# xxxupeng/stereo_toolbox

Measured on AMD Instinct MI355X. Metric: stereo pairs/sec @ 540x960 D=192 (GwcNet_GC fwd+bwd), higher is better.
Workload: dtype f32; 1 GPU; GwcNet_GC(maxdisp=192) train step: fwd+bwd+allreduce+Adam, 576x960 pairs (reference pad_to_2x shape), batch 1/GPU, fp32, synthetic randn inputs, deterministic filler weights; global_batch=1, parallelism=dp1, grad_sync=none (single rank: flat fp32 buffer packed, no collective), launch=eager, optimizer=torch.optim.Adam(fused=True)

## Files before the change

include/stx_hip.h:

```cpp
#ifndef STX_HIP_H
#define STX_HIP_H
#ifdef __cplusplus
extern "C" {
#endif

const char* stx_last_error(void);
const char* stx_build_info(void);
int stx_get_tuning(const char* name);
int stx_set_tuning(const char* name, int value);

int stx_cost_volume_fwd(const float* Lg, const float* Rg, int Cg, int G, const float* Lc, const float* Rc, int Cc,
                        const float* scale, float* vol, int B, int H, int W, int D, int mask_left, void* stream);
int stx_group_normalize_fwd(const float* x, float* y, int B, int C, int G, int HW, float out_scale, void* stream);
int stx_group_normalize_bwd(const float* x, const float* gy, float* gx, int B, int C, int G, int HW, float out_scale, void* stream);
int stx_cost_volume_bwd(const float* gvol, const float* Lg, const float* Rg, int Cg, int G, int Cc, float* gLg,
                        float* gRg, float* gLc, float* gRc, int B, int H, int W, int D, int mask_left, void* stream);

int stx_head_fwd(const float* cost, float* disp, float* stats, int B, int Dc, int Hc, int Wc, int D, int H, int W,
                 void* stream);
long long stx_head_bwd_workspace_floats(int B, int Dc, int H, int W);
int stx_head_bwd(const float* gdisp, const float* cost, const float* disp, const float* stats, float* gcost,
                 float* workspace, int B, int Dc, int Hc, int Wc, int D, int H, int W, void* stream);
int stx_head_fwd2(const float* cost, float* disp, float* stats, int B, int Dc, int Hc, int Wc, int D, int H, int W,
                  int align_corners, void* stream);
int stx_head_bwd2(const float* gdisp, const float* cost, const float* disp, const float* stats, float* gcost,
                  float* workspace, int B, int Dc, int Hc, int Wc, int D, int H, int W, int align_corners, void* stream);
int stx_softargmax_fwd(const float* x, float* out, int B, int D, int HW, void* stream);
int stx_argmax_fwd(const float* x, long long* out, int B, int D, int HW, void* stream);
int stx_unimodal_fwd(const float* x, float* out, int B, int D, int HW, void* stream);
int stx_dominant_modal_fwd(const float* x, float* out, int B, int D, int HW, void* stream);
int stx_modal_fwd(const float* x, float* out, float* aux, int B, int D, int HW, int kind, void* stream);
int stx_modal_bwd(const float* g, const float* out, const float* aux, float* gx, int B, int D, int HW, void* stream);
int stx_split_mode(const float* x, float* mode, unsigned char* mask, int B, int D, int HW, void* stream);
int stx_softmax_d_fwd(const float* x, float* y, int B, int D, int HW, void* stream);

long long stx_conv3d_packed_floats(int K, int N, int T);
int stx_conv3d_pack_weight(const float* w, float* wp, int A, int B, int T, int mode, void* stream);
int stx_conv3d_fwd_blocks(int Do, int Ho, int Wo);
long long stx_conv3d_fwd_stat_rows(int B, int Di, int Hi, int Wi, int Cin, int Cout, int ks, int stride);
int stx_conv3d_fwd(const float* x, const float* wp, float* out, const float* scale, const float* bias,
                   const float* residual, float* stats, int B, int Di, int Hi, int Wi, int Cin, int Cout, int ks,
                   int stride, int relu, void* stream);
int stx_deconv3d_fwd_blocks(int Di, int Hi, int Wi);
int stx_deconv3d_fwd(const float* x, const float* wp, float* out, const float* scale, const float* bias,
                     const float* residual, float* stats, int B, int Di, int Hi, int Wi, int Cin, int Cout, int Do,
                     int Ho, int Wo, int relu, void* stream);
long long stx_conv3d_wgrad_workspace_floats(int B, int Dc, int Hc, int Wc, int CF, int CC, int ks, int stride);
int stx_conv3d_wgrad(const float* fine, const float* coarse, float* dw, float* workspace, int B, int Df, int Hf, int Wf,
                     int CF, int Dc, int Hc, int Wc, int CC, int ks, int stride, void* stream);

int stx_conv3d_wgrad_bn_supported(int B, int D, int H, int W, int CF, int CC);
int stx_conv3d_wgrad_bn(const float* x, const float* gy, const float* z, const float* scale, const float* shift, const float* mean,
                        const float* invstd, const float* gamma, const float* sums, float inv_n, int act, float* dz, float* dw,
                        float* workspace, int B, int D, int H, int W, int CF, int CC, void* stream);

int stx_conv2d_supported(int Cin, int Cout);
long long stx_conv2d_stat_rows(int groups);
int stx_conv2d_fwd(const float* x, const float* w, float* out, float* stats, int B, int H, int W, int Cin, int Cout, int dgrad,
                   int groups, void* stream);

int stx_conv3d_c1_fwd(const float* x, const float* w, const float* residual, float* out, int B, int D, int H, int W,
                      int Cin, void* stream);
long long stx_conv3d_c1_wgrad_workspace_floats(int Cin);
int stx_conv3d_c1_wgrad(const float* x, const float* gy, float* dw, float* workspace, int B, int D, int H, int W,
                        int Cin, void* stream);
int stx_conv3d_c1_dgrad(const float* gy, const float* w, float* gx, int B, int D, int H, int W, int Cin, void* stream);

int stx_mish_fwd(const float* x, float* y, long long n, void* stream);
int stx_mish_bwd(const float* gy, const float* x, float* gx, long long n, void* stream);
int stx_depth_to_space(const float* y, float* out, int B, int D, int H, int W, int C, int inverse, void* stream);
int stx_gate_fwd(const float* cv, const float* att, float* out, int B, int D, long long HW, int C, void* stream);
int stx_gate_bwd(const float* g, const float* cv, const float* att, float* gcv, float* gatt, int B, int D, long long HW,
                 int C, void* stream);

int stx_concat_channels(const float* in0, const float* in1, const float* in2, const float* in3, int C0, int C1, int C2, int C3,
                        float* out, long long nvox, void* stream);
int stx_split_channels(const float* in, float* out0, float* out1, float* out2, float* out3, int C0, int C1, int C2, int C3,
                       long long nvox, void* stream);
int stx_transpose(const float* in, float* out, int N, int rows, int cols, void* stream);

int stx_dwconv_hw_fwd(const float* x, const float* w, const int* dil, float* out, int B, int D, int H, int W, int C,
                      int flip, void* stream);
long long stx_dwconv_hw_wgrad_workspace_floats(int C);
int stx_dwconv_hw_wgrad(const float* x, const float* gy, const int* dil, float* dw, float* workspace, int B, int D,
                        int H, int W, int C, void* stream);
int stx_cost_volume_scale_bwd(const float* gvol, const float* Lc, const float* Rc, float* gscale, int B, int Cc, int H,
                              int W, int D, int mask_left, void* stream);
int stx_scale_channels(const float* x, const float* s, float* out, long long nvox, int C, void* stream);
int stx_ac_volume_bwd(const float* gvol, const float* Lc, const float* Rc, const float* prob, float* gL, float* gR,
                      float* gprob, int B, int Cc, int H, int W, int D, int mask_left, void* stream);

int stx_bn_reduce_blocks(void);
int stx_bn_stats_rows(long long nvox, int C);
int stx_bn_stats(const float* z, float* partials, long long nvox, int C, int groups, void* stream);
int stx_bn_finalize(const float* partials, int nrows, int C, double count, const float* gamma, const float* beta,
                    float* running_mean, float* running_var, float momentum, float eps, float* scale, float* shift,
                    float* mean, float* invstd, void* stream);
int stx_bn_finalize_groups(const float* partials, int nrows, int C, double count, const float* gamma, const float* beta,
                           float* running_mean, float* running_var, float momentum, float eps, float* out, int groups,
                           void* stream);
int stx_bn_apply(const float* z1, const float* scale1, const float* shift1, const float* z2, const float* scale2,
                 const float* shift2, float* out, long long nvox, int C, int relu, int groups, void* stream);
int stx_bn_bwd_reduce(const float* gy, const float* y, const float* z1, const float* mean1, const float* invstd1,
                      const float* z2, const float* mean2, const float* invstd2, float* partials, float* sums,
                      long long nvox, int C, int relu, void* stream);
int stx_bn_bwd_apply(const float* gy, const float* y, const float* z1, const float* mean1, const float* invstd1,
                     const float* gamma1, const float* z2, const float* mean2, const float* invstd2,
                     const float* gamma2, const float* sums, float* dz1, float* dz2, float* gout, long long nvox, int C,
                     int relu, void* stream);
int stx_bn_bwd_reduce2(const float* gy, const float* y, const float* z1, const float* mean1, const float* invstd1,
                       const float* z2, const float* mean2, const float* invstd2, const float* scale1,
                       const float* shift1, const float* scale2, const float* shift2, float* partials, float* sums,
                       long long nvox, int C, int relu, int groups, void* stream);
int stx_bn_bwd_apply2(const float* gy, const float* y, const float* z1, const float* mean1, const float* invstd1,
                      const float* gamma1, const float* z2, const float* mean2, const float* invstd2,
                      const float* gamma2, const float* scale1, const float* shift1, const float* scale2,
                      const float* shift2, const float* sums, float* dz1, float* dz2, float* gout, long long nvox,
                      int C, int relu, int groups, void* stream);

int stx_pad_normalize_u8(const unsigned char* img, float* out, int B, int H, int W, int Hp, int Wp, int top,
                         const float* mean3, const float* std3, void* stream);

int stx_sampled_volume_fwd(const float* Lg, const float* Rg, int Cg, int G, const float* Lc, const float* Rc, int Cc,
                           const float* samples, float* vol, int B, int H, int W, int S, int CTp, void* stream);
int stx_sampled_volume_bwd(const float* gvol, const float* Lg, const float* Rg, int Cg, int G, int Cc,
                           const float* samples, float* gLg, float* gRg, float* gLc, float* gRc, int B, int H, int W,
                           int S, int CTp, void* stream);

int stx_warp_fwd(const float* x, const float* disp, float* out, int B, int C, int H, int W, void* stream);
int stx_warp_bwd(const float* gout, const float* x, const float* disp, float* gx, float* gdisp, int B, int C, int H, int W,
                 void* stream);
int stx_corr_volume_fwd(const float* ref, const float* tgt, float* vol, int B, int C, int H, int W, int maxdisp, int groups,
                        void* stream);
int stx_corr_volume_bwd(const float* gvol, const float* ref, const float* tgt, float* gref, float* gtgt, int B, int C, int H,
                        int W, int maxdisp, int groups, void* stream);
int stx_disparity_variance_fwd(const float* x, const float* disp, const float* samples, float* out, int B, int D, int HW,
                               void* stream);
int stx_disparity_variance_bwd(const float* g, const float* x, const float* disp, const float* samples, float* gx, float* gdisp,
                               float* gsamples, int B, int D, int HW, void* stream);

long long stx_geo_pyramid_floats(long long rows, int len, int C, int levels);
int stx_geo_corr_fwd(const float* fmap1, const float* fmap2, float* cpyr, int B, int C, int H, int W1, int W2, int levels,
                     void* stream);
int stx_geo_corr_bwd(const float* gcpyr, const float* fmap1, const float* fmap2, float* gfmap1, float* gfmap2, int B, int C, int H,
                     int W1, int W2, int levels, void* stream);
int stx_geo_pyramid_fwd(const float* vol, float* gpyr, int B, int D, int H, int W, int C, int levels, void* stream);
int stx_geo_pyramid_bwd(const float* ggpyr, float* gvol, int B, int D, int H, int W, int C, int levels, void* stream);
int stx_geo_lookup_fwd(const float* gpyr, const float* cpyr, const float* disp, const float* coords, float* out, int B, int H,
                       int W, int D, int C, int W2, int levels, int radius, void* stream);
int stx_geo_lookup_bwd(const float* gout, const float* disp, const float* coords, float* ggpyr, float* gcpyr, int B, int H, int W,
                       int D, int C, int W2, int levels, int radius, void* stream);
int stx_context_upsample_fwd(const float* disp_low, const float* up_weights, float* out, int B, int h, int w, void* stream);
int stx_context_upsample_bwd(const float* g, const float* disp_low, const float* up_weights, float* gdisp, float* gweights, int B,
                             int h, int w, void* stream);

long long stx_corr1d_pyramid_floats(long long rows, int W2, int levels);
int stx_corr1d_pyramid_fwd(const float* fmap1, const float* fmap2, float* cpyr, int B, int C, int H, int W1, int W2, int levels,
                           float scale, void* stream);
int stx_corr1d_pyramid_bwd(const float* gcpyr, const float* fmap1, const float* fmap2, float* gfmap1, float* gfmap2, int B, int C,
                           int H, int W1, int W2, int levels, float scale, void* stream);
int stx_corr1d_lookup_fwd(const float* cpyr, const float* base, const float* disp, const float* jobs, int njobs, float* out, int B,
                          int H, int W1, int W2, int levels, void* stream);
int stx_corr1d_lookup_bwd(const float* gout, const float* base, const float* disp, const float* jobs, int njobs, float* gcpyr,
                          int B, int H, int W1, int W2, int levels, void* stream);

int stx_allpairs_estimates_fwd(const float* vol, int which, float* disp_l, float* conf_l, float* disp_r, float* conf_r, float* stats,
                               int B, int H, int W1, int W2, void* stream);
int stx_allpairs_estimates_bwd(const float* g_disp_l, const float* g_conf_l, const float* g_disp_r, const float* g_conf_r,
                               const float* vol, const float* stats, float* gvol, int B, int H, int W1, int W2, void* stream);
int stx_corr1d_volume_pyramid_fwd(const float* vol, const float* tdisp, const float* tconf, float atten, float* cpyr, int B, int H,
                                  int W1, int W2, int levels, void* stream);
int stx_corr1d_volume_pyramid_bwd(const float* gcpyr, const float* tdisp, const float* tconf, float atten, float* gvol, int B, int H,
                                  int W1, int W2, int levels, void* stream);
int stx_truncate_mask_fwd(const float* disp, const float* conf, int has_th, float conf_th, float atten, float* mask, int B, int H,
                          int W, void* stream);

int stx_photo_warp_fwd(const float* right, const float* disp, float* warped, float* valid, int B, int C, int H, int W, void* stream);
int stx_photo_warp_bwd(const float* gwarped, const float* right, const float* disp, float* gdisp, int B, int C, int H, int W,
                       void* stream);
int stx_ssim_fwd(const float* x, const float* y, float* out, int B, int C, int H, int W, int window, void* stream);
long long stx_ssim_bwd_workspace_floats(int B, int C, int H, int W);
int stx_ssim_bwd(const float* g_out, const float* x, const float* y, float* gx, float* gy, float* workspace, int B, int C, int H, int W,
                 int window, void* stream);
int stx_photometric_fwd(const float* left, const float* right, const float* disp, double ssim_weight, int enable_mask, float* loss,
                        int B, int C, int H, int W, void* stream);
long long stx_photometric_bwd_workspace_floats(int B, int C, int H, int W);
int stx_photometric_bwd(const float* gloss, const float* left, const float* right, const float* disp, double ssim_weight,
                        int enable_mask, float* gdisp, float* workspace, int B, int C, int H, int W, void* stream);
int stx_auto_mask_fwd(const float* left, const float* right, const float* disp, int denorm, unsigned char* mask, int B, int C, int H,
                      int W, void* stream);
long long stx_smoothness_workspace_floats(int B, int H, int W);
int stx_smoothness_fwd(const float* disp, const float* img, float* out, float* stats, float* workspace, int B, int C, int H, int W,
                       void* stream);
int stx_smoothness_bwd(const float* gout, const float* disp, const float* img, const float* stats, float* gdisp, int B, int C, int H,
                       int W, void* stream);

int stx_sttr_head_fwd(const float* attn, const float* phi, int mode, int iters, float log_one, float log_bin, float log_2w,
                      const unsigned char* occ_mask, const float* target, float* disp, float* occ, float* norm, int* arg,
                      float* gt_response, float* bin_left, float* bin_right, double* us, double* vs, int N, int H, int W, void* stream);
int stx_sttr_head_bwd(const float* g_disp, const float* g_occ, const float* g_gt, const float* g_bin_left, const float* g_bin_right,
                      const float* attn, const float* phi, int mode, int iters, float log_one, float log_bin, float log_2w,
                      const float* target, const float* disp, const float* norm, const int* arg, const double* us, const double* vs,
                      float* g_attn, double* phi_partials, float* g_phi, int N, int H, int W, void* stream);
int stx_sttr_transport_fwd(const float* attn, const float* phi, int mode, int iters, float log_one, float log_bin, float log_2w,
                           float* P, double* us, double* vs, int N, int H, int W, void* stream);
int stx_sttr_transport_bwd(const float* G, const float* attn, const float* phi, int mode, int iters, float log_one, float log_bin,
                           float log_2w, const double* us, const double* vs, float* g_attn, double* phi_partials, float* g_phi, int N,
                           int H, int W, void* stream);

#ifdef __cplusplus
}
#endif
#endif
```

stereo_toolbox_amd/_capi.py:

```python
import ctypes
import os
import threading

import torch

_P = ctypes.c_void_p
_I = ctypes.c_int
_F = ctypes.c_float
_L = ctypes.c_longlong

SIGNATURES = {
    "stx_get_tuning": [ctypes.c_char_p],
    "stx_set_tuning": [ctypes.c_char_p, _I],
    "stx_cost_volume_fwd": [_P, _P, _I, _I, _P, _P, _I, _P, _P, _I, _I, _I, _I, _I, _P],
    "stx_cost_volume_bwd": [_P, _P, _P, _I, _I, _I, _P, _P, _P, _P, _I, _I, _I, _I, _I, _P],
    "stx_group_normalize_fwd": [_P, _P, _I, _I, _I, _I, _F, _P],
    "stx_group_normalize_bwd": [_P, _P, _P, _I, _I, _I, _I, _F, _P],
    "stx_head_fwd": [_P, _P, _P, _I, _I, _I, _I, _I, _I, _I, _P],
    "stx_head_bwd_workspace_floats": [_I, _I, _I, _I],
    "stx_head_bwd": [_P, _P, _P, _P, _P, _P, _I, _I, _I, _I, _I, _I, _I, _P],
    "stx_head_fwd2": [_P, _P, _P, _I, _I, _I, _I, _I, _I, _I, _I, _P],
    "stx_head_bwd2": [_P, _P, _P, _P, _P, _P, _I, _I, _I, _I, _I, _I, _I, _I, _P],
    "stx_softargmax_fwd": [_P, _P, _I, _I, _I, _P],
    "stx_argmax_fwd": [_P, _P, _I, _I, _I, _P],
    "stx_softmax_d_fwd": [_P, _P, _I, _I, _I, _P],
    "stx_unimodal_fwd": [_P, _P, _I, _I, _I, _P],
    "stx_dominant_modal_fwd": [_P, _P, _I, _I, _I, _P],
    "stx_modal_fwd": [_P, _P, _P, _I, _I, _I, _I, _P],
    "stx_modal_bwd": [_P, _P, _P, _P, _I, _I, _I, _P],
    "stx_split_mode": [_P, _P, _P, _I, _I, _I, _P],
    "stx_conv3d_packed_floats": [_I, _I, _I],
    "stx_conv3d_pack_weight": [_P, _P, _I, _I, _I, _I, _P],
    "stx_conv3d_fwd_blocks": [_I, _I, _I],
    "stx_conv3d_fwd_stat_rows": [_I, _I, _I, _I, _I, _I, _I, _I],
    "stx_deconv3d_fwd_blocks": [_I, _I, _I],
    "stx_conv3d_fwd": [_P, _P, _P, _P, _P, _P, _P, _I, _I, _I, _I, _I, _I, _I, _I, _I, _P],
    "stx_deconv3d_fwd": [_P, _P, _P, _P, _P, _P, _P, _I, _I, _I, _I, _I, _I, _I, _I, _I, _I, _P],
    "stx_conv3d_wgrad_workspace_floats": [_I, _I, _I, _I, _I, _I, _I, _I],
    "stx_conv3d_wgrad": [_P, _P, _P, _P, _I, _I, _I, _I, _I, _I, _I, _I, _I, _I, _I, _P],
    "stx_conv3d_wgrad_bn_supported": [_I, _I, _I, _I, _I, _I],
    "stx_conv3d_wgrad_bn": [_P] * 9 + [_F, _I, _P, _P, _P, _I, _I, _I, _I, _I, _I, _P],
    "stx_conv2d_supported": [_I, _I],
    "stx_conv2d_stat_rows": [_I],
    "stx_conv2d_fwd": [_P, _P, _P, _P, _I, _I, _I, _I, _I, _I, _I, _P],
    "stx_conv3d_c1_fwd": [_P, _P, _P, _P, _I, _I, _I, _I, _I, _P],
    "stx_conv3d_c1_wgrad_workspace_floats": [_I],
    "stx_conv3d_c1_wgrad": [_P, _P, _P, _P, _I, _I, _I, _I, _I, _P],
    "stx_conv3d_c1_dgrad": [_P, _P, _P, _I, _I, _I, _I, _I, _P],
    "stx_mish_fwd": [_P, _P, _L, _P],
    "stx_mish_bwd": [_P, _P, _P, _L, _P],
    "stx_depth_to_space": [_P, _P, _I, _I, _I, _I, _I, _I, _P],
    "stx_gate_fwd": [_P, _P, _P, _I, _I, _L, _I, _P],
    "stx_gate_bwd": [_P, _P, _P, _P, _P, _I, _I, _L, _I, _P],
    "stx_concat_channels": [_P, _P, _P, _P, _I, _I, _I, _I, _P, _L, _P],
    "stx_split_channels": [_P, _P, _P, _P, _P, _I, _I, _I, _I, _L, _P],
    "stx_transpose": [_P, _P, _I, _I, _I, _P],
    "stx_dwconv_hw_fwd": [_P, _P, _P, _P, _I, _I, _I, _I, _I, _I, _P],
    "stx_dwconv_hw_wgrad_workspace_floats": [_I],
    "stx_dwconv_hw_wgrad": [_P, _P, _P, _P, _P, _I, _I, _I, _I, _I, _P],
    "stx_cost_volume_scale_bwd": [_P, _P, _P, _P, _I, _I, _I, _I, _I, _I, _P],
    "stx_scale_channels": [_P, _P, _P, _L, _I, _P],
    "stx_ac_volume_bwd": [_P, _P, _P, _P, _P, _P, _P, _I, _I, _I, _I, _I, _I, _P],
    "stx_pad_normalize_u8": [_P, _P, _I, _I, _I, _I, _I, _I, _P, _P, _P],
    "stx_warp_fwd": [_P, _P, _P, _I, _I, _I, _I, _P],
    "stx_warp_bwd": [_P, _P, _P, _P, _P, _I, _I, _I, _I, _P],
    "stx_corr_volume_fwd": [_P, _P, _P, _I, _I, _I, _I, _I, _I, _P],
    "stx_corr_volume_bwd": [_P, _P, _P, _P, _P, _I, _I, _I, _I, _I, _I, _P],
    "stx_disparity_variance_fwd": [_P, _P, _P, _P, _I, _I, _I, _P],
    "stx_disparity_variance_bwd": [_P, _P, _P, _P, _P, _P, _P, _I, _I, _I, _P],
    "stx_sampled_volume_fwd": [_P, _P, _I, _I, _P, _P, _I, _P, _P, _I, _I, _I, _I, _I, _P],
    "stx_sampled_volume_bwd": [_P, _P, _P, _I, _I, _I, _P, _P, _P, _P, _P, _I, _I, _I, _I, _I, _P],
    "stx_geo_pyramid_floats": [_L, _I, _I, _I],
    "stx_geo_corr_fwd": [_P, _P, _P, _I, _I, _I, _I, _I, _I, _P],
    "stx_geo_corr_bwd": [_P, _P, _P, _P, _P, _I, _I, _I, _I, _I, _I, _P],
    "stx_geo_pyramid_fwd": [_P, _P, _I, _I, _I, _I, _I, _I, _P],
    "stx_geo_pyramid_bwd": [_P, _P, _I, _I, _I, _I, _I, _I, _P],
    "stx_geo_lookup_fwd": [_P, _P, _P, _P, _P, _I, _I, _I, _I, _I, _I, _I, _I, _P],
    "stx_geo_lookup_bwd": [_P, _P, _P, _P, _P, _I, _I, _I, _I, _I, _I, _I, _I, _P],
    "stx_context_upsample_fwd": [_P, _P, _P, _I, _I, _I, _P],
    "stx_context_upsample_bwd": [_P, _P, _P, _P, _P, _I, _I, _I, _P],
    "stx_corr1d_pyramid_floats": [_L, _I, _I],
    "stx_corr1d_pyramid_fwd": [_P, _P, _P, _I, _I, _I, _I, _I, _I, _F, _P],
    "stx_corr1d_pyramid_bwd": [_P, _P, _P, _P, _P, _I, _I, _I, _I, _I, _I, _F, _P],
    "stx_corr1d_lookup_fwd": [_P, _P, _P, _P, _I, _P, _I, _I, _I, _I, _I, _P],
    "stx_corr1d_lookup_bwd": [_P, _P, _P, _P, _I, _P, _I, _I, _I, _I, _I, _P],
    "stx_allpairs_estimates_fwd": [_P, _I, _P, _P, _P, _P, _P, _I, _I, _I, _I, _P],
    "stx_allpairs_estimates_bwd": [_P, _P, _P, _P, _P, _P, _P, _I, _I, _I, _I, _P],
    "stx_corr1d_volume_pyramid_fwd": [_P, _P, _P, _F, _P, _I, _I, _I, _I, _I, _P],
    "stx_corr1d_volume_pyramid_bwd": [_P, _P, _P, _F, _P, _I, _I, _I, _I, _I, _P],
    "stx_truncate_mask_fwd": [_P, _P, _I, _F, _F, _P, _I, _I, _I, _P],
    "stx_photo_warp_fwd": [_P, _P, _P, _P, _I, _I, _I, _I, _P],
    "stx_photo_warp_bwd": [_P, _P, _P, _P, _I, _I, _I, _I, _P],
    "stx_ssim_fwd": [_P, _P, _P, _I, _I, _I, _I, _I, _P],
    "stx_ssim_bwd_workspace_floats": [_I, _I, _I, _I],
    "stx_ssim_bwd": [_P, _P, _P, _P, _P, _P, _I, _I, _I, _I, _I, _P],
    "stx_photometric_fwd": [_P, _P, _P, ctypes.c_double, _I, _P, _I, _I, _I, _I, _P],
    "stx_photometric_bwd_workspace_floats": [_I, _I, _I, _I],
    "stx_photometric_bwd": [_P, _P, _P, _P, ctypes.c_double, _I, _P, _P, _I, _I, _I, _I, _P],
    "stx_auto_mask_fwd": [_P, _P, _P, _I, _P, _I, _I, _I, _I, _P],
    "stx_smoothness_workspace_floats": [_I, _I, _I],
    "stx_smoothness_fwd": [_P, _P, _P, _P, _P, _I, _I, _I, _I, _P],
    "stx_smoothness_bwd": [_P, _P, _P, _P, _P, _I, _I, _I, _I, _P],
    "stx_sttr_head_fwd": [_P, _P, _I, _I, _F, _F, _F] + [_P] * 11 + [_I, _I, _I, _P],
    "stx_sttr_head_bwd": [_P] * 7 + [_I, _I, _F, _F, _F] + [_P] * 9 + [_I, _I, _I, _P],
    "stx_sttr_transport_fwd": [_P, _P, _I, _I, _F, _F, _F, _P, _P, _P, _I, _I, _I, _P],
    "stx_sttr_transport_bwd": [_P, _P, _P, _I, _I, _F, _F, _F, _P, _P, _P, _P, _P, _I, _I, _I, _P],
    "stx_bn_reduce_blocks": [],
    "stx_bn_stats_rows": [_L, _I],
    "stx_bn_stats": [_P, _P, _L, _I, _I, _P],
    "stx_bn_finalize": [_P, _I, _I, ctypes.c_double, _P, _P, _P, _P, _F, _F, _P, _P, _P, _P, _P],
    "stx_bn_finalize_groups": [_P, _I, _I, ctypes.c_double, _P, _P, _P, _P, _F, _F, _P, _I, _P],
    "stx_bn_apply": [_P, _P, _P, _P, _P, _P, _P, _L, _I, _I, _I, _P],
    "stx_bn_bwd_reduce": [_P, _P, _P, _P, _P, _P, _P, _P, _P, _P, _L, _I, _I, _P],
    "stx_bn_bwd_apply": [_P, _P, _P, _P, _P, _P, _P, _P, _P, _P, _P, _P, _P, _P, _L, _I, _I, _P],
    "stx_bn_bwd_reduce2": [_P] * 14 + [_L, _I, _I, _I, _P],
    "stx_bn_bwd_apply2": [_P] * 18 + [_L, _I, _I, _I, _P],
}
_RET_CHARP = ("stx_last_error", "stx_build_info")


class StxError(RuntimeError):
    pass


class StxLib:

    def __init__(self, path):
        if not os.path.exists(path):
            raise StxError(
                f"HIP library not found: {path}. Build it with `python -m stereo_toolbox_amd.build` "
                "(hipcc, gfx950). There is no CPU fallback for the cost-volume hot path.")
        self.path = path
        self._dll = ctypes.CDLL(path)
        for name in _RET_CHARP:
            fn = getattr(self._dll, name)
            fn.restype = ctypes.c_char_p
            fn.argtypes = []
        self._fns = {}
        for name, argtypes in SIGNATURES.items():
            fn = getattr(self._dll, name, None)
            if fn is None:
                continue
            fn.restype = ctypes.c_longlong if name.endswith(("_floats", "_stat_rows")) else _I
            fn.argtypes = argtypes
            self._fns[name] = fn

    def has(self, name):
        return name in self._fns

    def build_info(self):
        return self._dll.stx_build_info().decode()

    def get_tuning(self, name):
        return self._fns["stx_get_tuning"](name.encode())

    def set_tuning(self, name, value):
        old = self.get_tuning(name)
        if old < 0 or self._fns["stx_set_tuning"](name.encode(), int(value)) != 0:
            raise StxError(f"unknown tuning switch {name}")
        return old

    def raw(self, name):
        return self._fns[name]

    def call(self, name, *args):
        fn = self._fns.get(name)
        if fn is None:
            raise StxError(f"{self.path} does not export {name}")
        rc = fn(*args)
        if rc != 0:
            raise StxError(f"{name} failed ({rc}): {self._dll.stx_last_error().decode()}")


_LIB = None
_LOCK = threading.Lock()
LIB_PATH = os.environ.get("STX_HIP_LIB") or os.path.join(os.path.dirname(os.path.abspath(__file__)), "lib", "libstx_hip.so")


def get_lib():
    global _LIB
    if _LIB is None:
        with _LOCK:
            if _LIB is None:
                _LIB = StxLib(LIB_PATH)
    return _LIB
```

stereo_toolbox_amd/aggregation.py:

```python
import os
import threading

import torch
import torch.nn as nn

from . import ops


def _is_transposed(conv):
    return isinstance(conv, nn.ConvTranspose3d)


def _conv_cfg(conv):
    ks = conv.kernel_size[0]
    stride = conv.stride[0]
    if _is_transposed(conv):
        k3 = ks == 3 and stride == 2 and conv.padding[0] == 1 and conv.output_padding[0] == 1
        k4 = ks == 4 and stride == 2 and conv.padding[0] == 1 and conv.output_padding[0] == 0
        if not (k3 or k4) or len(set(conv.kernel_size)) != 1 or len(set(conv.stride)) != 1:
            raise ops.StxError("only ConvTranspose3d(k=3, s=2, p=1, op=1) and ConvTranspose3d(k=4, s=2, p=1) are on the hot path")
    else:
        if not ((ks == 3 and conv.padding[0] == 1 and stride in (1, 2)) or (ks == 1 and conv.padding[0] == 0 and stride == 1)):
            raise ops.StxError(f"unsupported Conv3d k={ks} s={stride} p={conv.padding}")
    if conv.bias is not None or conv.groups != 1:
        raise ops.StxError("hot-path convolutions are bias-free and dense")
    return ks, stride


def _fold(bn):
    key = (bn.weight._version, bn.bias._version, bn.running_mean._version, bn.running_var._version,
           bn.weight.data_ptr(), bn.bias.data_ptr(), bn.running_mean.data_ptr(), bn.running_var.data_ptr())
    hit = bn.__dict__.get("_stx_fold") if ops._CACHE_ENABLED else None
    if hit is not None and hit[0] == key:
        return hit[1], hit[2]
    with torch.no_grad():
        scale = (bn.weight * torch.rsqrt(bn.running_var + bn.eps)).contiguous()
        bias = (bn.bias - bn.running_mean * scale).contiguous()
    if ops._CACHE_ENABLED:
        bn.__dict__["_stx_fold"] = (key, scale, bias)
    return scale, bias


def _needs_grad(*tensors_and_modules):
    if not torch.is_grad_enabled():
        return False
    for t in tensors_and_modules:
        if t is None:
            continue
        if isinstance(t, torch.Tensor):
            if t.requires_grad:
                return True
        else:
            if any(p.requires_grad for p in t.parameters()):
                return True
    return False


def _infer_conv(x, conv, scale, bias, residual, relu):
    ks, stride = _conv_cfg(conv)
    if _is_transposed(conv) and ks == 4:
        if residual is not None:
            raise ops.StxError("ConvTranspose3d(k4) with a fused residual is not wired (no model uses it)")
        return ops.deconv4_forward(x, conv.weight.detach(), scale, bias, int(relu), owner=conv.weight)
    if _is_transposed(conv):
        wp = ops.pack_weight(conv.weight.detach(), 2, owner=conv.weight)
        return ops.deconv3d_forward(x, wp, conv.weight.shape[1], scale=scale, bias=bias, residual=residual, relu=relu)[0]
    if ops._is_c1(conv.weight, ks, stride, False) and scale is None and bias is None and not relu:
        return ops.conv3d_c1_forward(x, conv.weight.detach().contiguous(), residual)
    if x.shape[-1] != conv.weight.shape[1]:
        if x.shape[-1] != (conv.weight.shape[1] + 7) // 8 * 8:
            raise ops.StxError(f"conv: input has {x.shape[-1]} channels, weight expects {conv.weight.shape[1]}")
        wpad = ops.pad_weight_channels(conv.weight.detach(), x.shape[-1])
        return ops.conv3d_forward(x, ops.pack_weight(wpad, 0), conv.weight.shape[0], ks, stride, scale, bias, residual, relu)[0]
    if x.shape[-1] % 8 != 0:
        xp, wpad = ops.pad_input_channels(x, conv.weight.detach())
        return ops.conv3d_forward(xp, ops.pack_weight(wpad, 0), conv.weight.shape[0], ks, stride, scale, bias, residual, relu)[0]
    wp = ops.pack_weight(conv.weight.detach(), 0, owner=conv.weight)
    return ops.conv3d_forward(x, wp, conv.weight.shape[0], ks, stride, scale, bias, residual, relu)[0]


class deferred_bn_counters:
    _tls = threading.local()

    @staticmethod
    def _state():
        st = deferred_bn_counters._tls
        if not hasattr(st, "active"):
            st.active, st.pending = 0, []
        return st

    def __enter__(self):
        self._state().active += 1
        ops.bn_defer_reset_if_stale()
        return self

    def __exit__(self, *exc):
        st = self._state()
        st.active -= 1
        if st.active == 0 and st.pending:
            pend, st.pending = st.pending, []
            by_dev = {}
            for t in pend:
                d = by_dev.setdefault(t.device, {})
                ent = d.setdefault(id(t), [t, 0])
                ent[1] += 1
            for d in by_dev.values():
                torch._foreach_add_([e[0] for e in d.values()], [e[1] for e in d.values()])
        return False


def _bn_state(bn, partials, count, steps=1):
    training = bn.training
    sync = None
    if training and isinstance(bn, nn.SyncBatchNorm):
        import torch.distributed as dist
        if dist.is_available() and dist.is_initialized() and dist.get_world_size(bn.process_group) > 1:
            sync = (bn.process_group, dist.get_world_size(bn.process_group))
    if training:
        bn.__dict__.pop("_stx_fold", None)
    if training and bn.track_running_stats and bn.num_batches_tracked is not None:
        st = deferred_bn_counters._state()
        if st.active and bn.momentum is not None:
            st.pending.extend([bn.num_batches_tracked] * steps)
        else:
            bn.num_batches_tracked.add_(steps)
    if bn.momentum is not None:
        momentum = bn.momentum
    elif training and bn.track_running_stats and bn.num_batches_tracked is not None:
        momentum = 1.0 / float(bn.num_batches_tracked.item())
    else:
        momentum = 0.0
    return {"training": training, "partials": partials, "count": count, "running_mean": bn.running_mean,
            "running_var": bn.running_var, "momentum": momentum, "eps": bn.eps, "sync": sync}


def _raw_conv(x, conv, want):
    ks, stride = _conv_cfg(conv)
    if _is_transposed(conv) and ks == 4:
        return ops.deconv4_raw(x, conv.weight, want)
    return ops.ConvRawFn.apply(x, conv.weight, ks, stride, _is_transposed(conv), want)


@ops.fp32_region
def shared_input_convs(x, blocks):
    cfgs, ws = [], []
    for seq in blocks:
        conv, bn = seq[0], seq[1]
        if _is_transposed(conv) or not bn.training or conv.weight.shape[1] != x.shape[-1] or conv.weight.shape[1] % 8 \
                or conv.weight.shape[0] % 8:
            return None
        ks, stride = _conv_cfg(conv)
        cfgs.append((ks, stride, True))
        ws.append(conv.weight)
    if not _needs_grad(x, *[m for seq in blocks for m in (seq[0], seq[1])]):
        return None
    outs = ops.SharedInputConvsFn.apply(x, tuple(cfgs), *ws)
    return [(outs[2 * k], outs[2 * k + 1]) for k in range(len(blocks))]


@ops.fp32_region
def conv_block(x, conv, bn=None, relu=False, second=None, residual=None, mish=False, leaky=False, raw=None, second_raw=None):
    if (mish and relu) or (leaky and (relu or mish)):
        raise ops.StxError("conv_block: relu, mish and leaky are mutually exclusive")
    if second is not None and residual is not None:
        raise ops.StxError("conv_block: `second` and `residual` are mutually exclusive")
    mods = [conv, bn] + ([second[1], second[2]] if second is not None else [])
    grad = (raw is not None or second_raw is not None
            or _needs_grad(x, residual, *(m for m in mods if m is not None), *([second[0]] if second else [])))
    train_bn = (bn is not None and bn.training) or (second is not None and second[2].training)
    if mish and (grad or train_bn) and (bn is None or residual is not None):
        return ops.mish(conv_block(x, conv, bn, relu=False, second=second, residual=residual))
    if mish:
        relu = 2
    if leaky:
        relu = 3

    if not grad and not train_bn:
        if second is not None:
            s2, b2 = _fold(second[2])
            residual = _infer_conv(second[0], second[1], s2, b2, None, False)
        if bn is not None:
            s1, b1 = _fold(bn)
        else:
            s1 = b1 = None
        return _infer_conv(x, conv, s1, b1, residual, relu)

    want = bn is not None and bn.training
    z1, part1 = raw if raw is not None else _raw_conv(x, conv, want)
    if bn is None:
        y = z1
        if residual is not None:
            y = y + residual
        if relu == 3:
            return torch.nn.functional.leaky_relu(y, 0.01)
        return torch.relu(y) if relu else y
    count1 = z1.numel() // z1.shape[-1]
    st1 = _bn_state(bn, part1 if want else None, count1)
    if second is not None:
        x2, conv2, bn2 = second
        want2 = bn2.training
        z2, part2 = second_raw if second_raw is not None else _raw_conv(x2, conv2, want2)
        st2 = _bn_state(bn2, part2 if want2 else None, z2.numel() // z2.shape[-1])
        return ops.BnActFn.apply(z1, bn.weight, bn.bias, z2, bn2.weight, bn2.bias, None, relu, st1, st2)
    defer = (residual is None and want and relu in (0, 1, False, True) and not _is_transposed(conv) and _conv_cfg(conv) == (3, 1)
             and conv.weight.shape[0] % 32 == 0 and conv.weight.shape[1] % 32 == 0 and not st1.get("sync")
             and os.environ.get("STX_BN_BWD_IN_WGRAD", "1") != "0")
    if defer:
        ops.bn_defer_reset_if_stale()
    return ops.BnActFn.apply(z1, bn.weight, bn.bias, None, None, None, residual, relu, st1, None, 1, defer)


@ops.fp32_region
def convbn_block(x, seq, relu=False, second=None, residual=None, mish=False, raw=None, second_raw=None):
    sec = None
    if second is not None:
        sec = (second[0], second[1][0], second[1][1])
    return conv_block(x, seq[0], seq[1], relu=relu, second=sec, residual=residual, mish=mish, raw=raw, second_raw=second_raw)
```

stereo_toolbox_amd/csrc/bn.hip:

```cpp
#include "stx_common.h"
#include <stdlib.h>

namespace {

constexpr int BN_THREADS = 256;
constexpr int BN_RED_BLOCKS = 1024;

__device__ __forceinline__ double bn_block_sum(double v, double* red, int tid) {
    red[tid] = v;
    __syncthreads();
    for (int s = BN_THREADS / 2; s > 0; s >>= 1) {
        if (tid < s) red[tid] += red[tid + s];
        __syncthreads();
    }
    const double r = red[0];
    __syncthreads();
    return r;
}

__global__ __launch_bounds__(BN_THREADS) void bn_finalize_kernel(
    const float* __restrict__ partials, int nrows, int C, double count, const float* __restrict__ gamma,
    const float* __restrict__ beta, float* __restrict__ running_mean, float* __restrict__ running_var,
    float momentum, float eps, float* __restrict__ scale, float* __restrict__ shift, float* __restrict__ mean_out,
    float* __restrict__ invstd_out, int groups) {
// ... 107 lines not shown
                u.z = fmaf(u.z, a2.z, b2.z); u.w = fmaf(u.w, a2.w, b2.w);
            }
            v.x += u.x; v.y += u.y; v.z += u.z; v.w += u.w;
        }
        if (relu) {
            v.x = stx_act(v.x, relu); v.y = stx_act(v.y, relu); v.z = stx_act(v.z, relu); v.w = stx_act(v.w, relu);
        }
        stx_st4(out + i * 4, v);
    }
}

__global__ __launch_bounds__(BN_THREADS) void bn_bwd_reduce_kernel(
    const float* __restrict__ gy, const float* __restrict__ y, const float* __restrict__ z1,
    const float* __restrict__ mean1, const float* __restrict__ invstd1, const float* __restrict__ z2,
    const float* __restrict__ mean2, const float* __restrict__ invstd2, const float* __restrict__ sc1,
    const float* __restrict__ sh1, const float* __restrict__ sc2, const float* __restrict__ sh2, float* __restrict__ partials,
    size_t nvox, int C, int relu) {
    __shared__ float red[BN_THREADS * 12];
    const int tid = threadIdx.x;
    const int CQ = C >> 2;
    const int cq = tid % CQ, vl = tid / CQ, VPB = BN_THREADS / CQ;
    {
        const size_t go = (size_t)blockIdx.y * nvox * C, gc = (size_t)blockIdx.y * C;
        gy += go; z1 += go; mean1 += gc; invstd1 += gc;
        if (y) y += go;
        if (z2) z2 += go;
        if (mean2) { mean2 += gc; invstd2 += gc; }
        if (sc1) { sc1 += gc; sh1 += gc; }
        if (sc2) { sc2 += gc; sh2 += gc; }
        partials += (size_t)blockIdx.y * gridDim.x * 3 * C;
    }
    const float4 m1 = stx_ld4(mean1 + 4 * cq), i1 = stx_ld4(invstd1 + 4 * cq);
    float4 m2 = make_float4(0.f, 0.f, 0.f, 0.f), i2 = m2;
    const bool has2 = z2 && mean2;
    if (has2) { m2 = stx_ld4(mean2 + 4 * cq); i2 = stx_ld4(invstd2 + 4 * cq); }
    const bool remask = relu && !y;
    float4 a1 = m2, b1 = m2, a2 = m2, b2 = m2;
    if (remask) {
        a1 = stx_ld4(sc1 + 4 * cq); b1 = stx_ld4(sh1 + 4 * cq);
        if (has2) { a2 = stx_ld4(sc2 + 4 * cq); b2 = stx_ld4(sh2 + 4 * cq); }
    }
    float s[12];
#pragma unroll
    for (int k = 0; k < 12; ++k) s[k] = 0.f;
    for (size_t v = vl < VPB ? (size_t)blockIdx.x * VPB + vl : nvox; v < nvox; v += (size_t)gridDim.x * VPB) {
        const size_t o = v * C + 4 * cq;
        float4 g = stx_ld4(gy + o);
        const float4 a = stx_ld4(z1 + o);
        float4 c = make_float4(0.f, 0.f, 0.f, 0.f);
        if (has2) c = stx_ld4(z2 + o);
        if (relu) {
            float4 yy;
            if (remask) {
                yy.x = fmaf(a.x, a1.x, b1.x); yy.y = fmaf(a.y, a1.y, b1.y); yy.z = fmaf(a.z, a1.z, b1.z); yy.w = fmaf(a.w, a1.w, b1.w);
                if (has2) {
                    yy.x += fmaf(c.x, a2.x, b2.x); yy.y += fmaf(c.y, a2.y, b2.y);
                    yy.z += fmaf(c.z, a2.z, b2.z); yy.w += fmaf(c.w, a2.w, b2.w);
                }
            } else {
                yy = stx_ld4(y + o);
            }
            g.x = stx_act_bwd(g.x, yy.x, relu); g.y = stx_act_bwd(g.y, yy.y, relu);
            g.z = stx_act_bwd(g.z, yy.z, relu); g.w = stx_act_bwd(g.w, yy.w, relu);
        }
        s[0] += g.x; s[1] += g.y; s[2] += g.z; s[3] += g.w;
        s[4] = fmaf(g.x, (a.x - m1.x) * i1.x, s[4]); s[5] = fmaf(g.y, (a.y - m1.y) * i1.y, s[5]);
        s[6] = fmaf(g.z, (a.z - m1.z) * i1.z, s[6]); s[7] = fmaf(g.w, (a.w - m1.w) * i1.w, s[7]);
        if (has2) {
            s[8] = fmaf(g.x, (c.x - m2.x) * i2.x, s[8]); s[9] = fmaf(g.y, (c.y - m2.y) * i2.y, s[9]);
            s[10] = fmaf(g.z, (c.z - m2.z) * i2.z, s[10]); s[11] = fmaf(g.w, (c.w - m2.w) * i2.w, s[11]);
        }
    }
#pragma unroll
    for (int k = 0; k < 12; ++k) red[k * BN_THREADS + tid] = s[k];
    __syncthreads();
    for (int idx = tid; idx < 12 * CQ; idx += BN_THREADS) {
        const int k = idx / CQ, q = idx % CQ;
        float t = 0.f;
        for (int j = q; j < BN_THREADS; j += CQ) t += red[k * BN_THREADS + j];
        partials[((size_t)blockIdx.x * 3 + (k >> 2)) * C + 4 * q + (k & 3)] = t;
    }
}

__global__ __launch_bounds__(BN_THREADS) void bn_stats_kernel(const float* __restrict__ z, float* __restrict__ partials,
                                                              size_t nvox, int C) {
    __shared__ float red[BN_THREADS * 8];
    const int tid = threadIdx.x;
    const int CQ = C >> 2;
    const int cq = tid % CQ, vl = tid / CQ, VPB = BN_THREADS / CQ;
    z += (size_t)blockIdx.y * nvox * C;
    partials += (size_t)blockIdx.y * gridDim.x * 2 * C;
    float s[8];
#pragma unroll
    for (int k = 0; k < 8; ++k) s[k] = 0.f;
    const size_t step = (size_t)gridDim.x * VPB;
    size_t v = vl < VPB ? (size_t)blockIdx.x * VPB + vl : nvox;
    for (; v + 3 * step < nvox; v += 4 * step) {
        float4 a[4];
#pragma unroll
        for (int u = 0; u < 4; ++u) a[u] = stx_ld4(z + (v + u * step) * C + 4 * cq);
#pragma unroll
        for (int u = 0; u < 4; ++u) {
            s[0] += a[u].x; s[1] += a[u].y; s[2] += a[u].z; s[3] += a[u].w;
            s[4] = fmaf(a[u].x, a[u].x, s[4]); s[5] = fmaf(a[u].y, a[u].y, s[5]);
            s[6] = fmaf(a[u].z, a[u].z, s[6]); s[7] = fmaf(a[u].w, a[u].w, s[7]);
        }
    }
    for (; v < nvox; v += step) {
        const float4 a = stx_ld4(z + v * C + 4 * cq);
        s[0] += a.x; s[1] += a.y; s[2] += a.z; s[3] += a.w;
        s[4] = fmaf(a.x, a.x, s[4]); s[5] = fmaf(a.y, a.y, s[5]); s[6] = fmaf(a.z, a.z, s[6]); s[7] = fmaf(a.w, a.w, s[7]);
    }
#pragma unroll
    for (int k = 0; k < 8; ++k) red[k * BN_THREADS + tid] = s[k];
    __syncthreads();
    for (int idx = tid; idx < 8 * CQ; idx += BN_THREADS) {
        const int k = idx / CQ, q = idx % CQ;
        float t = 0.f;
        for (int j = q; j < BN_THREADS; j += CQ) t += red[k * BN_THREADS + j];
        partials[((size_t)blockIdx.x * 2 + (k >> 2)) * C + 4 * q + (k & 3)] = t;
    }
}

__global__ __launch_bounds__(BN_THREADS) void bn_colsum_kernel(const float* __restrict__ partials, int nrows, int M,
                                                               float* __restrict__ sums, int groups) {
    __shared__ double red[BN_THREADS];
    const int m = blockIdx.x, tid = threadIdx.x;
    float tot = 0.f;
    for (int g = 0; g < groups; ++g) {
        const float* p = partials + (size_t)g * nrows * M;
        double s = 0.0;
        for (int r = tid; r < nrows; r += BN_THREADS) s += (double)p[(size_t)r * M + m];
        s = bn_block_sum(s, red, tid);
        if (tid == 0) {
            sums[(size_t)g * M + m] = (float)s;
            tot += (float)s;
        }
    }
    if (groups > 1 && tid == 0) sums[(size_t)groups * M + m] = tot;
}

__global__ __launch_bounds__(BN_THREADS) void bn_bwd_apply_kernel(
    const float* __restrict__ gy, const float* __restrict__ y, const float* __restrict__ z1,
    const float* __restrict__ mean1, const float* __restrict__ invstd1, const float* __restrict__ gamma1,
    const float* __restrict__ z2, const float* __restrict__ mean2, const float* __restrict__ invstd2,
    const float* __restrict__ gamma2, const float* __restrict__ sc1, const float* __restrict__ sh1,
    const float* __restrict__ sc2, const float* __restrict__ sh2, const float* __restrict__ sums, float* __restrict__ dz1,
    float* __restrict__ dz2, float* __restrict__ gout, size_t nquads, int C, int relu, float inv_n) {
    const int CQ = C >> 2;
    {
        const size_t go = (size_t)blockIdx.y * nquads * 4, gc = (size_t)blockIdx.y * C;
        gy += go; z1 += go; dz1 += go; mean1 += gc; invstd1 += gc; sums += 3 * gc;
        if (y) y += go;
        if (z2) z2 += go;
        if (dz2) dz2 += go;
        if (gout) gout += go;
        if (mean2) { mean2 += gc; invstd2 += gc; }
        if (sc1) { sc1 += gc; sh1 += gc; }
        if (sc2) { sc2 += gc; sh2 += gc; }
    }
    const bool has2 = z2 && mean2 && dz2;
    const bool remask = relu && !y;
    for (size_t i = (size_t)blockIdx.x * BN_THREADS + threadIdx.x; i < nquads; i += (size_t)gridDim.x * BN_THREADS) {
        const int c = (int)(i % CQ) * 4;
        float4 g = stx_ld4(gy + i * 4);
        const float4 a = stx_ld4(z1 + i * 4);
        float4 a2v = make_float4(0.f, 0.f, 0.f, 0.f);
        if (has2) a2v = stx_ld4(z2 + i * 4);
        if (relu) {
            float4 yy;
            if (remask) {
                const float4 p1 = stx_ld4(sc1 + c), q1 = stx_ld4(sh1 + c);
                yy.x = fmaf(a.x, p1.x, q1.x); yy.y = fmaf(a.y, p1.y, q1.y); yy.z = fmaf(a.z, p1.z, q1.z); yy.w = fmaf(a.w, p1.w, q1.w);
                if (has2) {
                    const float4 p2 = stx_ld4(sc2 + c), q2 = stx_ld4(sh2 + c);
                    yy.x += fmaf(a2v.x, p2.x, q2.x); yy.y += fmaf(a2v.y, p2.y, q2.y);
                    yy.z += fmaf(a2v.z, p2.z, q2.z); yy.w += fmaf(a2v.w, p2.w, q2.w);
                }
            } else {
                yy = stx_ld4(y + i * 4);
            }
            g.x = stx_act_bwd(g.x, yy.x, relu); g.y = stx_act_bwd(g.y, yy.y, relu);
            g.z = stx_act_bwd(g.z, yy.z, relu); g.w = stx_act_bwd(g.w, yy.w, relu);
        }
        if (gout) stx_st4(gout + i * 4, g);
        const float4 sg = stx_ld4(sums + c);
        {
            const float4 m = stx_ld4(mean1 + c), is = stx_ld4(invstd1 + c);
            const float4 gm = gamma1 ? stx_ld4(gamma1 + c) : make_float4(1.f, 1.f, 1.f, 1.f);
            const float4 sx = stx_ld4(sums + C + c);
            float4 d;
            d.x = gm.x * is.x * (g.x - sg.x * inv_n - (a.x - m.x) * is.x * sx.x * inv_n);
            d.y = gm.y * is.y * (g.y - sg.y * inv_n - (a.y - m.y) * is.y * sx.y * inv_n);
            d.z = gm.z * is.z * (g.z - sg.z * inv_n - (a.z - m.z) * is.z * sx.z * inv_n);
            d.w = gm.w * is.w * (g.w - sg.w * inv_n - (a.w - m.w) * is.w * sx.w * inv_n);
            stx_st4(dz1 + i * 4, d);
        }
        if (has2) {
            const float4 a = a2v, m = stx_ld4(mean2 + c), is = stx_ld4(invstd2 + c);
            const float4 gm = gamma2 ? stx_ld4(gamma2 + c) : make_float4(1.f, 1.f, 1.f, 1.f);
            const float4 sx = stx_ld4(sums + 2 * C + c);
            float4 d;
            d.x = gm.x * is.x * (g.x - sg.x * inv_n - (a.x - m.x) * is.x * sx.x * inv_n);
            d.y = gm.y * is.y * (g.y - sg.y * inv_n - (a.y - m.y) * is.y * sx.y * inv_n);
            d.z = gm.z * is.z * (g.z - sg.z * inv_n - (a.z - m.z) * is.z * sx.z * inv_n);
            d.w = gm.w * is.w * (g.w - sg.w * inv_n - (a.w - m.w) * is.w * sx.w * inv_n);
            stx_st4(dz2 + i * 4, d);
        }
    }
}

int bn_grid(size_t nquads) {
    size_t g = (nquads + BN_THREADS - 1) / BN_THREADS;
    return (int)(g > 4096 ? 4096 : (g < 1 ? 1 : g));
}

}

extern "C" int stx_bn_reduce_blocks(void) {
    stx_begin(); return BN_RED_BLOCKS; }

static int bn_finalize_launch(const float* partials, int nrows, int C, double count, const float* gamma, const float* beta,
                              float* running_mean, float* running_var, float momentum, float eps, float* scale, float* shift,
                              float* mean, float* invstd, int groups, void* stream) {
    if (C % 4 == 0 && nrows >= 256)
        hipLaunchKernelGGL(bn_finalize4_kernel, dim3(C / 4), dim3(BN_FIN_THREADS), 0, (hipStream_t)stream, partials, nrows, C,
                           count, gamma, beta, running_mean, running_var, momentum, eps, scale, shift, mean, invstd, groups);
    else
        hipLaunchKernelGGL(bn_finalize_kernel, dim3(C), dim3(BN_THREADS), 0, (hipStream_t)stream, partials, nrows, C, count,
                           gamma, beta, running_mean, running_var, momentum, eps, scale, shift, mean, invstd, groups);
    return stx_check_launch("bn_finalize");
}

extern "C" int stx_bn_finalize(const float* partials, int nrows, int C, double count, const float* gamma,
                               const float* beta, float* running_mean, float* running_var, float momentum, float eps,
                               float* scale, float* shift, float* mean, float* invstd, void* stream) {
    stx_begin();
    STX_REQUIRE(partials && nrows > 0 && C > 0 && count > 0 && scale && shift && mean && invstd, "bn_finalize: bad args");
    return bn_finalize_launch(partials, nrows, C, count, gamma, beta, running_mean, running_var, momentum, eps, scale, shift,
                              mean, invstd, 1, stream);
}

extern "C" int stx_bn_finalize_groups(const float* partials, int nrows, int C, double count, const float* gamma,
                                      const float* beta, float* running_mean, float* running_var, float momentum, float eps,
                                      float* out, int groups, void* stream) {
    stx_begin();
    STX_REQUIRE(partials && nrows > 0 && C > 0 && count > 0 && out && groups >= 1, "bn_finalize_groups: bad args");
    const size_t gc = (size_t)groups * C;
    return bn_finalize_launch(partials, nrows, C, count, gamma, beta, running_mean, running_var, momentum, eps, out, out + gc,
                              out + 2 * gc, out + 3 * gc, groups, stream);
}

extern "C" int stx_bn_stats_rows(long long nvox, int C) {
    stx_begin();
    if (C < 4 || C % 4 != 0 || C / 4 > BN_THREADS || nvox < 1) return 0;
    const long long vpb = BN_THREADS / (C / 4);
    const long long g = (nvox + 4 * vpb - 1) / (4 * vpb);
    return (int)(g > 256 ? 256 : (g < 1 ? 1 : g));
}

extern "C" int stx_bn_stats(const float* z, float* partials, long long nvox, int C, int groups, void* stream) {
    stx_begin();
    STX_REQUIRE(z && partials && nvox > 0 && groups >= 1 && groups <= 65535, "bn_stats: bad args");
    STX_REQUIRE(C >= 4 && C % 4 == 0 && C / 4 <= BN_THREADS, "bn_stats: C=%d unsupported (a multiple of 4, at most 1024)", C);
    hipLaunchKernelGGL(bn_stats_kernel, dim3(stx_bn_stats_rows(nvox, C), groups), dim3(BN_THREADS), 0, (hipStream_t)stream, z,
                       partials, (size_t)nvox, C);
    return stx_check_launch("bn_stats");
}

extern "C" int stx_bn_apply(const float* z1, const float* scale1, const float* shift1, const float* z2,
                            const float* scale2, const float* shift2, float* out, long long nvox, int C, int relu,
                            int groups, void* stream) {
    stx_begin();
    STX_REQUIRE(z1 && scale1 && shift1 && out && nvox > 0 && C > 0 && C % 4 == 0, "bn_apply: bad args (C=%d)", C);
    STX_REQUIRE(!scale2 || (z2 && shift2), "bn_apply: second affine needs z2 and shift2");
    STX_REQUIRE(groups >= 1 && groups <= 65535, "bn_apply: groups=%d", groups);
    const size_t nquads = (size_t)nvox * (C / 4);
    hipLaunchKernelGGL(bn_apply_kernel, dim3(bn_grid(nquads), groups), dim3(BN_THREADS), 0, (hipStream_t)stream, z1, scale1,
                       shift1, z2, scale2, shift2, out, nquads, C / 4, relu);
    return stx_check_launch("bn_apply");
}

extern "C" int stx_bn_bwd_reduce2(const float* gy, const float* y, const float* z1, const float* mean1,
                                  const float* invstd1, const float* z2, const float* mean2, const float* invstd2,
                                  const float* scale1, const float* shift1, const float* scale2, const float* shift2,
                                  float* partials, float* sums, long long nvox, int C, int relu, int groups, void* stream) {
    stx_begin();
    STX_REQUIRE(gy && z1 && mean1 && invstd1 && partials && sums && nvox > 0, "bn_bwd_reduce: null operand");
    STX_REQUIRE(groups >= 1 && groups <= 65535, "bn_bwd_reduce: groups=%d", groups);
    STX_REQUIRE(C >= 4 && C % 4 == 0 && C / 4 <= BN_THREADS, "bn_bwd_reduce: C=%d unsupported (a multiple of 4, at most 1024)", C);
    STX_REQUIRE(!relu || y || (scale1 && shift1 && (!(z2 && mean2) || (scale2 && shift2))),
                "bn_bwd_reduce: the relu mask needs y or the forward pass's scale / shift vectors");
    STX_REQUIRE(relu != 2 || !y, "bn_bwd_reduce: Mish (activation code 2) differentiates the pre-activation value: pass y = NULL and the scale / shift vectors");
    hipStream_t st = (hipStream_t)stream;
    const int nblk = ((long long)nvox * C <= (9ll << 19)) ? BN_RED_BLOCKS / 4 : BN_RED_BLOCKS;
    hipLaunchKernelGGL(bn_bwd_reduce_kernel, dim3(nblk, groups), dim3(BN_THREADS), 0, st, gy, y, z1, mean1, invstd1,
                       z2, mean2, invstd2, scale1, shift1, scale2, shift2, partials, (size_t)nvox, C, relu);
    int rc = stx_check_launch("bn_bwd_reduce");
    if (rc) return rc;
    hipLaunchKernelGGL(bn_colsum_kernel, dim3(3 * C), dim3(BN_THREADS), 0, st, partials, nblk, 3 * C, sums, groups);
    return stx_check_launch("bn_colsum");
}

extern "C" int stx_bn_bwd_apply2(const float* gy, const float* y, const float* z1, const float* mean1,
                                 const float* invstd1, const float* gamma1, const float* z2, const float* mean2,
                                 const float* invstd2, const float* gamma2, const float* scale1, const float* shift1,
                                 const float* scale2, const float* shift2, const float* sums, float* dz1, float* dz2,
                                 float* gout, long long nvox, int C, int relu, int groups, void* stream) {
    stx_begin();
    STX_REQUIRE(gy && z1 && mean1 && invstd1 && sums && dz1 && nvox > 0 && C % 4 == 0, "bn_bwd_apply: bad args");
    STX_REQUIRE(groups >= 1 && groups <= 65535, "bn_bwd_apply: groups=%d", groups);
    STX_REQUIRE(!relu || y || (scale1 && shift1 && (!(z2 && mean2 && dz2) || (scale2 && shift2))),
                "bn_bwd_apply: the relu mask needs y or the forward pass's scale / shift vectors");
    STX_REQUIRE(relu != 2 || !y, "bn_bwd_apply: Mish (activation code 2) differentiates the pre-activation value: pass y = NULL and the scale / shift vectors");
    const size_t nquads = (size_t)nvox * (C / 4);
    hipLaunchKernelGGL(bn_bwd_apply_kernel, dim3(bn_grid(nquads), groups), dim3(BN_THREADS), 0, (hipStream_t)stream, gy, y, z1,
                       mean1, invstd1, gamma1, z2, mean2, invstd2, gamma2, scale1, shift1, scale2, shift2, sums, dz1, dz2,
                       gout, nquads, C, relu, (float)(1.0 / (double)nvox));
    return stx_check_launch("bn_bwd_apply");
}

extern "C" int stx_bn_bwd_reduce(const float* gy, const float* y, const float* z1, const float* mean1,
                                 const float* invstd1, const float* z2, const float* mean2, const float* invstd2,
                                 float* partials, float* sums, long long nvox, int C, int relu, void* stream) {
    return stx_bn_bwd_reduce2(gy, y, z1, mean1, invstd1, z2, mean2, invstd2, nullptr, nullptr, nullptr, nullptr, partials,
                              sums, nvox, C, relu, 1, stream);
}

extern "C" int stx_bn_bwd_apply(const float* gy, const float* y, const float* z1, const float* mean1,
                                const float* invstd1, const float* gamma1, const float* z2, const float* mean2,
                                const float* invstd2, const float* gamma2, const float* sums, float* dz1, float* dz2,
                                float* gout, long long nvox, int C, int relu, void* stream) {
    return stx_bn_bwd_apply2(gy, y, z1, mean1, invstd1, gamma1, z2, mean2, invstd2, gamma2, nullptr, nullptr, nullptr,
                             nullptr, sums, dz1, dz2, gout, nvox, C, relu, 1, stream);
}
```

stereo_toolbox_amd/csrc/conv_c1.hip:

```cpp
#include "stx_common.h"
#include <stdlib.h>

namespace {

constexpr int C1_THREADS = 256;
constexpr int C1_TD = 2, C1_TH = 4, C1_TW = 32;
constexpr int C1_ED = C1_TD + 2, C1_EH = C1_TH + 2, C1_EW = C1_TW + 2;
constexpr int C1_CK = 16, C1_VS = C1_CK + 4;

struct C1Args {
    const float* x;
    const float* w;
    const float* gy;
    const float* res;
    float* out;
    int B, D, H, W, Cin;
    int nDt, nHt, nWt, ntiles;
};

__device__ __forceinline__ void c1_stage(const C1Args& a, float* tile, int b, int d0, int h0, int w0, int c0, int tid) {
    for (int idx = tid; idx < C1_ED * C1_EH * C1_EW * (C1_CK / 4); idx += C1_THREADS) {
        const int v = idx / (C1_CK / 4), f = idx - v * (C1_CK / 4);
        const int wx = v % C1_EW, hy = (v / C1_EW) % C1_EH, dz = v / (C1_EW * C1_EH);
        const int gd = d0 - 1 + dz, gh = h0 - 1 + hy, gw = w0 - 1 + wx;
        float4 val = make_float4(0.f, 0.f, 0.f, 0.f);
        if (gd >= 0 && gd < a.D && gh >= 0 && gh < a.H && gw >= 0 && gw < a.W)
            val = stx_ld4(a.x + ((((size_t)b * a.D + gd) * a.H + gh) * a.W + gw) * a.Cin + c0 + 4 * f);
        stx_st4(tile + v * C1_VS + 4 * f, val);
    }
}

__global__ __launch_bounds__(C1_THREADS) void conv_c1_fwd_kernel(C1Args a) {
    STX_DYN_SMEM(smem);
    float* tile = reinterpret_cast<float*>(smem);
    const int tid = threadIdx.x;
    int r = blockIdx.x;
    const int wt = r % a.nWt; r /= a.nWt;
    const int ht = r % a.nHt; r /= a.nHt;
    const int dt = r % a.nDt;
    const int b = r / a.nDt;
    const int d0 = dt * C1_TD, h0 = ht * C1_TH, w0 = wt * C1_TW;
    const int lw = tid % C1_TW, lh = (tid / C1_TW) % C1_TH, ld = tid / (C1_TW * C1_TH);
    const int base = ((ld * C1_EH + lh) * C1_EW + lw) * C1_VS;
    float acc = 0.f;
    for (int c0 = 0; c0 < a.Cin; c0 += C1_CK) {
        __syncthreads();
        c1_stage(a, tile, b, d0, h0, w0, c0, tid);
        __syncthreads();
        for (int tap = 0; tap < 27; ++tap) {
            const int kd = tap / 9, kh = (tap / 3) % 3, kw = tap % 3;
            const float* p = tile + base + ((kd * C1_EH + kh) * C1_EW + kw) * C1_VS;
#pragma unroll
            for (int f = 0; f < C1_CK / 4; ++f) {
                const float4 v = stx_ld4(p + 4 * f);
                const float* wp = a.w + (size_t)(c0 + 4 * f) * 27 + tap;
                acc = fmaf(v.x, wp[0], acc);
                acc = fmaf(v.y, wp[27], acc);
                acc = fmaf(v.z, wp[54], acc);
                acc = fmaf(v.w, wp[81], acc);
            }
        }
    }
    const int od = d0 + ld, oh = h0 + lh, ow = w0 + lw;
    if (od < a.D && oh < a.H && ow < a.W) {
        const size_t o = (((size_t)b * a.D + od) * a.H + oh) * a.W + ow;
        a.out[o] = a.res ? acc + a.res[o] : acc;
    }
}

__global__ __launch_bounds__(C1_THREADS) void conv_c1_wgrad_kernel(C1Args a) {
    STX_DYN_SMEM(smem);
    float* tile = reinterpret_cast<float*>(smem);
    float* gys = tile + C1_ED * C1_EH * C1_EW * C1_VS;
    const int tid = threadIdx.x;
    const int cl = tid & 15, tg = tid >> 4;
    const int nchunk = a.Cin / C1_CK;
    float acc[4][2];
#pragma unroll
    for (int i = 0; i < 4; ++i) { acc[i][0] = 0.f; acc[i][1] = 0.f; }
    const int tapA = tg, tapB = tg + 16;
    const int offA = (((tapA / 9) * C1_EH + (tapA / 3) % 3) * C1_EW + tapA % 3) * C1_VS + cl;
    const int tB = tapB < 27 ? tapB : 0;
    const int offB = (((tB / 9) * C1_EH + (tB / 3) % 3) * C1_EW + tB % 3) * C1_VS + cl;

    for (int t = blockIdx.x; t < a.ntiles; t += gridDim.x) {
        int r = t;
        const int wt = r % a.nWt; r /= a.nWt;
        const int ht = r % a.nHt; r /= a.nHt;
        const int dt = r % a.nDt;
        const int b = r / a.nDt;
        const int d0 = dt * C1_TD, h0 = ht * C1_TH, w0 = wt * C1_TW;
#pragma unroll
        for (int ck = 0; ck < 4; ++ck) {
            if (ck < nchunk) {
                __syncthreads();
                c1_stage(a, tile, b, d0, h0, w0, ck * C1_CK, tid);
                if (ck == 0) {
                    const int lw = tid % C1_TW, lh = (tid / C1_TW) % C1_TH, ld = tid / (C1_TW * C1_TH);
                    const int od = d0 + ld, oh = h0 + lh, ow = w0 + lw;
                    gys[tid] = (od < a.D && oh < a.H && ow < a.W)
                                   ? a.gy[(((size_t)b * a.D + od) * a.H + oh) * a.W + ow] : 0.f;
                }
                __syncthreads();
                float sA = 0.f, sB = 0.f;
                for (int v = 0; v < C1_TD * C1_TH * C1_TW; ++v) {
                    const int lw = v % C1_TW, lh = (v / C1_TW) % C1_TH, ld = v / (C1_TW * C1_TH);
                    const int vb = ((ld * C1_EH + lh) * C1_EW + lw) * C1_VS;
                    const float g = gys[v];
                    sA = fmaf(tile[vb + offA], g, sA);
                    sB = fmaf(tile[vb + offB], g, sB);
                }
                acc[ck][0] += sA;
                acc[ck][1] += sB;
            }
        }
    }
    float* dst = a.out + (size_t)blockIdx.x * a.Cin * 27;
#pragma unroll
    for (int ck = 0; ck < 4; ++ck) {
        if (ck < nchunk) {
            dst[(ck * C1_CK + cl) * 27 + tapA] = acc[ck][0];
            if (tapB < 27) dst[(ck * C1_CK + cl) * 27 + tapB] = acc[ck][1];
        }
    }
}

__global__ __launch_bounds__(C1_THREADS) void c1_colsum_kernel(const float* __restrict__ partials, int nrows, int M,
                                                               float* __restrict__ sums) {
    __shared__ double red[C1_THREADS];
    const int m = blockIdx.x, tid = threadIdx.x;
    double s = 0.0;
    for (int r = tid; r < nrows; r += C1_THREADS) s += (double)partials[(size_t)r * M + m];
    red[tid] = s;
    __syncthreads();
    for (int k = C1_THREADS / 2; k > 0; k >>= 1) {
        if (tid < k) red[tid] += red[tid + k];
        __syncthreads();
    }
    if (tid == 0) sums[m] = (float)red[0];
}

constexpr size_t C1_TILE_BYTES = (size_t)C1_ED * C1_EH * C1_EW * C1_VS * 4;
constexpr int C1_WGRAD_BLOCKS = 512;


constexpr int C1D_TH = 4, C1D_TW = 32;
constexpr int C1D_EH = C1D_TH + 2, C1D_EW = C1D_TW + 2;

__global__ __launch_bounds__(C1_THREADS) void conv_c1_dgrad_kernel(const float* __restrict__ gy,
                                                                   const float* __restrict__ w, float* __restrict__ gx,
                                                                   int B, int D, int H, int W, int Cin, int nHt, int nWt) {
    __shared__ float gys[3 * C1D_EH * C1D_EW];
    __shared__ float ws[27 * 64];
    const int tid = threadIdx.x;
    int r = blockIdx.x;
    const int wt = r % nWt; r /= nWt;
    const int ht = r % nHt; r /= nHt;
    const int d = r % D;
    const int b = r / D;
    const int h0 = ht * C1D_TH, w0 = wt * C1D_TW;
    for (int idx = tid; idx < 3 * C1D_EH * C1D_EW; idx += C1_THREADS) {
        const int wx = idx % C1D_EW, hy = (idx / C1D_EW) % C1D_EH, dz = idx / (C1D_EW * C1D_EH);
        const int gd = d - 1 + dz, gh = h0 - 1 + hy, gw = w0 - 1 + wx;
        gys[idx] = (gd >= 0 && gd < D && gh >= 0 && gh < H && gw >= 0 && gw < W)
                       ? gy[(((size_t)b * D + gd) * H + gh) * W + gw] : 0.f;
    }
    for (int idx = tid; idx < 27 * Cin; idx += C1_THREADS) {
        const int c = idx % Cin, tap = idx / Cin;
        ws[tap * Cin + c] = w[(size_t)c * 27 + tap];
    }
    __syncthreads();
    const int CQ = Cin >> 2;
    for (int item = tid; item < CQ * (C1D_TH * C1D_TW / 4); item += C1_THREADS) {
        const int q = item % CQ, grp = item / CQ;
        const int lw = (grp % (C1D_TW / 4)) * 4, lh = grp / (C1D_TW / 4);
        float4 acc[4];
#pragma unroll
        for (int j = 0; j < 4; ++j) acc[j] = make_float4(0.f, 0.f, 0.f, 0.f);
#pragma unroll
        for (int kd = 0; kd < 3; ++kd)
#pragma unroll
            for (int kh = 0; kh < 3; ++kh) {
                const float* gp = gys + (((2 - kd) * C1D_EH) + (lh + 2 - kh)) * C1D_EW + lw;
                float g6[6];
#pragma unroll
                for (int j = 0; j < 6; ++j) g6[j] = gp[j];
#pragma unroll
                for (int kw = 0; kw < 3; ++kw) {
                    const float4 wv = stx_ld4(ws + ((kd * 3 + kh) * 3 + kw) * Cin + 4 * q);
#pragma unroll
                    for (int j = 0; j < 4; ++j) {
                        const float g = g6[j + 2 - kw];
                        acc[j].x = fmaf(g, wv.x, acc[j].x);
                        acc[j].y = fmaf(g, wv.y, acc[j].y);
                        acc[j].z = fmaf(g, wv.z, acc[j].z);
                        acc[j].w = fmaf(g, wv.w, acc[j].w);
                    }
                }
            }
        const int oh = h0 + lh;
        if (oh < H) {
            float* o = gx + ((((size_t)b * D + d) * H + oh) * W + w0 + lw) * Cin + 4 * q;
#pragma unroll
            for (int j = 0; j < 4; ++j)
                if (w0 + lw + j < W) stx_st4(o + (size_t)j * Cin, acc[j]);
        }
    }
}


__global__ __launch_bounds__(C1_THREADS) void conv_c1_dgrad_mfma_kernel(const float* __restrict__ gy,
                                                                        const float* __restrict__ w, float* __restrict__ gx,
                                                                        int B, int D, int H, int W, int nHt, int nWt, int ntiles) {
    __shared__ float gys[3 * C1D_EH * C1D_EW];
    const int tid = threadIdx.x, lane = tid & 63, wave = tid >> 6;
    const int i = lane & 31, half = lane >> 5;
    float wreg[14];
    int aoff[14];
#pragma unroll
    for (int j = 0; j < 14; ++j) {
        const int tap = 2 * j + half;
        const int tp = tap < 27 ? tap : 26;
        const int kd = tp / 9, kh = (tp / 3) % 3, kw = tp % 3;
        wreg[j] = tap < 27 ? w[(size_t)i * 27 + tap] : 0.f;
        aoff[j] = ((2 - kd) * C1D_EH + (wave + 2 - kh)) * C1D_EW + i + 2 - kw;
    }
    const unsigned plane_bytes = (unsigned)H * (unsigned)W * 128u;
    for (int tile = blockIdx.x; tile < ntiles; tile += gridDim.x) {
        int r_ = tile;
        const int wt = r_ % nWt; r_ /= nWt;
        const int ht = r_ % nHt; r_ /= nHt;
        const int d = r_ % D;
        const int b = r_ / D;
        const int h0 = ht * C1D_TH, w0 = wt * C1D_TW;
        __syncthreads();
        for (int idx = tid; idx < 3 * C1D_EH * C1D_EW; idx += C1_THREADS) {
            const int wx = idx % C1D_EW, hy = (idx / C1D_EW) % C1D_EH, dz = idx / (C1D_EW * C1D_EH);
            const int gd = d - 1 + dz, gh = h0 - 1 + hy, gw = w0 - 1 + wx;
            gys[idx] = (gd >= 0 && gd < D && gh >= 0 && gh < H && gw >= 0 && gw < W)
                           ? gy[(((size_t)b * D + gd) * H + gh) * W + gw] : 0.f;
        }
        __syncthreads();
        f32x16 acc;
#pragma unroll
        for (int r = 0; r < 16; ++r) acc[r] = 0.f;
        float av[14];
#pragma unroll
        for (int j = 0; j < 14; ++j) av[j] = gys[aoff[j]];
#pragma unroll
        for (int j = 0; j < 14; ++j) acc = __builtin_amdgcn_mfma_f32_32x32x2f32(av[j], wreg[j], acc, 0, 0, 0);
        const int oh = h0 + wave;
        const stx_bufrsrc ors = stx_make_rsrc(gx + ((size_t)b * D + d) * H * W * 32, plane_bytes);
        const unsigned vbase = (unsigned)((((oh < H ? oh : 0) * W + w0 + 4 * half) * 32 + i) * 4);
#pragma unroll
        for (int r = 0; r < 16; ++r) {
            const int m = (r & 3) + 8 * (r >> 2);
            const bool ok = oh < H && w0 + 4 * half + m < W;
            stx_buf_st1(ors, ok ? vbase : STX_BUF_OOB, (unsigned)(m * 128), acc[r]);
        }
    }
}


constexpr int C1M_TD = 2, C1M_TH = 8, C1M_TW = 32;
constexpr int C1M_ED = C1M_TD + 2, C1M_EH = C1M_TH + 2, C1M_EW = C1M_TW + 2;
constexpr int C1M_BLOCKS = 1024;

__global__ __launch_bounds__(C1_THREADS) void conv_c1_wgrad_mfma_kernel(const float* __restrict__ x,
                                                                        const float* __restrict__ gy,
                                                                        float* __restrict__ slab, int B, int D, int H,
                                                                        int W, int Cin, int nDt, int nHt, int nWt,
                                                                        int ntiles) {
    __shared__ float gys[C1M_ED * C1M_EH * C1M_EW];
    __shared__ float red[4][1024];
    const int tid = threadIdx.x, lane = tid & 63, wave = tid >> 6;
    const int i = lane & 31, half = lane >> 5;
    const int cb = blockIdx.y;
    const int kd = i / 9, kh = (i / 3) % 3, kw = i % 3;
    const int toff = (i < 27) ? ((2 - kd) * C1M_EH + (2 - kh)) * C1M_EW + (2 - kw) + half : half;
    f32x16 acc;
#pragma unroll
    for (int r = 0; r < 16; ++r) acc[r] = 0.f;
    for (int t = blockIdx.x; t < ntiles; t += gridDim.x) {
        int r = t;
        const int wt = r % nWt; r /= nWt;
        const int ht = r % nHt; r /= nHt;
        const int dt = r % nDt;
        const int b = r / nDt;
        const int d0 = dt * C1M_TD, h0 = ht * C1M_TH, w0 = wt * C1M_TW;
        __syncthreads();
        for (int idx = tid; idx < C1M_ED * C1M_EH * C1M_EW; idx += C1_THREADS) {
            const int wx = idx % C1M_EW, hy = (idx / C1M_EW) % C1M_EH, dz = idx / (C1M_EW * C1M_EH);
            const int gd = d0 - 1 + dz, gh = h0 - 1 + hy, gw = w0 - 1 + wx;
            gys[idx] = (gd >= 0 && gd < D && gh >= 0 && gh < H && gw >= 0 && gw < W)
                           ? gy[(((size_t)b * D + gd) * H + gh) * W + gw] : 0.f;
        }
        __syncthreads();
#pragma unroll 1
        for (int k = 0; k < 4; ++k) {
            const int row = wave * 4 + k;
            const int ld = row / C1M_TH, lh = row % C1M_TH;
            const int gd = d0 + ld, gh = h0 + lh;
            const bool rowok = gd < D && gh < H;
            const float* xr = x + ((((size_t)b * D + gd) * H + gh) * W + w0 + half) * Cin + cb * 32 + i;
            float av[16];
#pragma unroll
            for (int p = 0; p < 16; ++p)
                av[p] = (rowok && w0 + 2 * p + half < W) ? xr[(size_t)(2 * p) * Cin] : 0.f;
            const float* gp = gys + (ld * C1M_EH + lh) * C1M_EW + toff;
#pragma unroll
            for (int p = 0; p < 16; ++p) {
                float bv = gp[2 * p];
                bv = (i < 27) ? bv : 0.f;
                acc = __builtin_amdgcn_mfma_f32_32x32x2f32(av[p], bv, acc, 0, 0, 0);
            }
        }
    }
#pragma unroll
    for (int r = 0; r < 16; ++r) red[wave][((r & 3) + 8 * (r >> 2) + 4 * half) * 32 + i] = acc[r];
    __syncthreads();
    float* dst = slab + ((size_t)cb * gridDim.x + blockIdx.x) * 1024;
    for (int idx = tid; idx < 1024; idx += C1_THREADS)
        dst[idx] = (red[0][idx] + red[1][idx]) + (red[2][idx] + red[3][idx]);
}

__global__ __launch_bounds__(C1_THREADS) void c1m_reduce_kernel(const float* __restrict__ slab, int nrows,
                                                                float* __restrict__ dw) {
    __shared__ double red[C1_THREADS];
    const int m = blockIdx.x, tid = threadIdx.x;
    const int tap = m % 27, cfull = m / 27, cb = cfull >> 5, c = cfull & 31;
    const float* p = slab + (size_t)cb * nrows * 1024 + c * 32 + tap;
    double s = 0.0;
    for (int r = tid; r < nrows; r += C1_THREADS) s += (double)p[(size_t)r * 1024];
    red[tid] = s;
    __syncthreads();
    for (int k = C1_THREADS / 2; k > 0; k >>= 1) {
        if (tid < k) red[tid] += red[tid + k];
        __syncthreads();
    }
    if (tid == 0) dw[m] = (float)red[0];
}


constexpr int C1F_TH = 8, C1F_TW = 32;
constexpr int C1F_EH = C1F_TH + 2, C1F_EW = C1F_TW + 2, C1F_NV = C1F_EH * C1F_EW;
constexpr int C1F_MT = (C1F_NV + 31) / 32;
constexpr int C1F_WGS = 512;

__global__ __launch_bounds__(C1_THREADS) void conv_c1_fwd_mfma_kernel(const float* __restrict__ x,
                                                                      const float* __restrict__ w,
                                                                      const float* __restrict__ res,
                                                                      float* __restrict__ out, int B, int D, int H, int W,
                                                                      int nHt, int nWt, int ncols) {
    STX_DYN_SMEM(smem);
    float* Ps = reinterpret_cast<float*>(smem);
    const int tid = threadIdx.x, lane = tid & 63, wave = __builtin_amdgcn_readfirstlane(tid >> 6);
    const int i = lane & 31, half = lane >> 5;
    float wreg[16];
#pragma unroll
    for (int s_ = 0; s_ < 16; ++s_) wreg[s_] = (i < 27) ? w[(size_t)(16 * half + s_) * 27 + i] : 0.f;
    const int lh = tid / C1F_TW, lw = tid % C1F_TW;

    constexpr int MTW = (C1F_MT + 3) / 4;
    const long long units = (long long)ncols * D;
    int u = __builtin_amdgcn_readfirstlane((int)(units * blockIdx.x / gridDim.x));
    const int u_end = __builtin_amdgcn_readfirstlane((int)(units * (blockIdx.x + 1) / gridDim.x));
    const unsigned plane_bytes = (unsigned)H * (unsigned)W * 32u * 4u;
    while (u < u_end) {
        const int col = u / D;
        const int d_lo = u - col * D;
        const int left = u_end - u;
        const int d_hi = (D - d_lo < left) ? D : d_lo + left;
        u += d_hi - d_lo;
        const int wt = col % nWt, ht = (col / nWt) % nHt, b = col / (nWt * nHt);
        const int h0 = ht * C1F_TH, w0 = wt * C1F_TW;
        const int oh = h0 + lh, ow = w0 + lw;
        const bool ook = oh < H && ow < W;
        unsigned voff[MTW];
#pragma unroll
        for (int t = 0; t < MTW; ++t) {
            const int hv = (wave + 4 * t) * 32 + i;
            const int hy = hv / C1F_EW, wx = hv - hy * C1F_EW;
            const int gh = h0 - 1 + hy, gw = w0 - 1 + wx;
            const bool ok = wave + 4 * t < C1F_MT && hv < C1F_NV && gh >= 0 && gh < H && gw >= 0 && gw < W;
            voff[t] = ok ? (unsigned)(((gh * W + gw) * 32 + 16 * half) * 4) : STX_BUF_OOB;
        }
        float4 nxt[MTW][4];
        auto load_plane = [&](int p) {
            const bool in = p >= 0 && p < D && p <= d_hi;
            const stx_bufrsrc rs = stx_make_rsrc(x + ((size_t)b * D + (in ? p : 0)) * H * W * 32, in ? plane_bytes : 0u);
#pragma unroll
            for (int t = 0; t < MTW; ++t)
#pragma unroll
                for (int q = 0; q < 4; ++q) nxt[t][q] = stx_buf_ld4(rs, voff[t], 16u * q);
        };
        float accA = 0.f, accB = 0.f;
        load_plane(d_lo - 1);
        __syncthreads();
        for (int p = d_lo - 1; p <= d_hi; ++p) {
            float* Pb = Ps + ((p + 2) & 1) * (C1F_NV * 27);
            const bool pin = p >= 0 && p < D;
            float4 cur[MTW][4];
#pragma unroll
            for (int t = 0; t < MTW; ++t)
#pragma unroll
                for (int q = 0; q < 4; ++q) cur[t][q] = nxt[t][q];
            load_plane(p + 1);
            if (pin) {
#pragma unroll
                for (int t = 0; t < MTW; ++t) {
                    const int m = wave + 4 * t;
                    if (m < C1F_MT) {
                        f32x16 acc;
#pragma unroll
                        for (int r = 0; r < 16; ++r) acc[r] = 0.f;
#pragma unroll
                        for (int q = 0; q < 4; ++q) {
                            acc = __builtin_amdgcn_mfma_f32_32x32x2f32(cur[t][q].x, wreg[4 * q + 0], acc, 0, 0, 0);
                            acc = __builtin_amdgcn_mfma_f32_32x32x2f32(cur[t][q].y, wreg[4 * q + 1], acc, 0, 0, 0);
                            acc = __builtin_amdgcn_mfma_f32_32x32x2f32(cur[t][q].z, wreg[4 * q + 2], acc, 0, 0, 0);
                            acc = __builtin_amdgcn_mfma_f32_32x32x2f32(cur[t][q].w, wreg[4 * q + 3], acc, 0, 0, 0);
                        }
                        if (i < 27) {
#pragma unroll
                            for (int r = 0; r < 16; ++r) {
                                const int v = m * 32 + (r & 3) + 8 * (r >> 2) + 4 * half;
                                if (v < C1F_NV) Pb[v * 27 + i] = acc[r];
                            }
                        }
                    }
                }
            }
            __syncthreads();
            float s0 = 0.f, s1 = 0.f, s2 = 0.f;
            if (pin) {
#pragma unroll
                for (int kh = 0; kh < 3; ++kh)
#pragma unroll
                    for (int kw = 0; kw < 3; ++kw) {
                        const float* pp = Pb + ((lh + kh) * C1F_EW + lw + kw) * 27 + kh * 3 + kw;
                        s0 += pp[0];
                        s1 += pp[9];
                        s2 += pp[18];
                    }
            }
            const float done = accA + s2;
            const int od = p - 1;
            if (od >= d_lo && od < d_hi && ook) {
                const size_t o = (((size_t)b * D + od) * H + oh) * W + ow;
                out[o] = res ? done + res[o] : done;
            }
            accA = accB + s1;
            accB = s0;
        }
    }
}

}

extern "C" int stx_conv3d_c1_fwd(const float* x, const float* w, const float* residual, float* out, int B, int D,
                                 int H, int W, int Cin, void* stream) {
    stx_begin();
    STX_REQUIRE(x && w && out && B > 0 && D > 0 && H > 0 && W > 0, "conv3d_c1_fwd: bad shape");
    STX_REQUIRE(Cin % C1_CK == 0, "conv3d_c1_fwd: Cin=%d must be a multiple of %d", Cin, C1_CK);
    if (Cin == 32 && (long long)H * W * 128 < (1ll << 31)) {
        const int nHt = stx_cdiv(H, C1F_TH), nWt = stx_cdiv(W, C1F_TW);
        const long long ncols = (long long)B * nHt * nWt, units = ncols * D;
        STX_REQUIRE(units < (1ll << 31), "conv3d_c1_fwd: volume too large");
        long long g = C1F_WGS;
        if (g > units / 4) g = units / 4 > 0 ? units / 4 : 1;
        const size_t lds = (size_t)2 * C1F_NV * 27 * 4;
        if (int rc = stx_lds_require((const void*)conv_c1_fwd_mfma_kernel, lds, "conv3d_c1_fwd(mfma)")) return rc;
        hipLaunchKernelGGL(conv_c1_fwd_mfma_kernel, dim3((unsigned)g), dim3(C1_THREADS), lds, (hipStream_t)stream, x, w,
                           residual, out, B, D, H, W, nHt, nWt, (int)ncols);
        return stx_check_launch("conv3d_c1_fwd(mfma)");
    }
    C1Args a;
    a.x = x; a.w = w; a.gy = nullptr; a.res = residual; a.out = out;
    a.B = B; a.D = D; a.H = H; a.W = W; a.Cin = Cin;
    a.nDt = stx_cdiv(D, C1_TD); a.nHt = stx_cdiv(H, C1_TH); a.nWt = stx_cdiv(W, C1_TW);
    a.ntiles = B * a.nDt * a.nHt * a.nWt;
    if (int rc = stx_lds_require((const void*)conv_c1_fwd_kernel, C1_TILE_BYTES, "conv3d_c1_fwd")) return rc;
    hipLaunchKernelGGL(conv_c1_fwd_kernel, dim3(a.ntiles), dim3(C1_THREADS), C1_TILE_BYTES, (hipStream_t)stream, a);
    return stx_check_launch("conv3d_c1_fwd");
}

extern "C" long long stx_conv3d_c1_wgrad_workspace_floats(int Cin) {
    const long long valu = (long long)C1_WGRAD_BLOCKS * Cin * 27;
    const long long mfma = (long long)C1M_BLOCKS * 1024 * ((Cin + 31) / 32);
    return valu > mfma ? valu : mfma;
}

extern "C" int stx_conv3d_c1_wgrad(const float* x, const float* gy, float* dw, float* workspace, int B, int D, int H,
                                   int W, int Cin, void* stream) {
    stx_begin();
    STX_REQUIRE(x && gy && dw && workspace && B > 0, "conv3d_c1_wgrad: null operand");
    STX_REQUIRE(Cin % C1_CK == 0 && Cin <= 4 * C1_CK, "conv3d_c1_wgrad: Cin=%d must be 16..64 in steps of 16", Cin);
    if (Cin % 32 == 0) {
        const int nDt = stx_cdiv(D, C1M_TD), nHt = stx_cdiv(H, C1M_TH), nWt = stx_cdiv(W, C1M_TW);
        const long long nt = (long long)B * nDt * nHt * nWt;
        STX_REQUIRE(nt < (1ll << 31), "conv3d_c1_wgrad: volume too large");
        const int nblk = nt < C1M_BLOCKS ? (int)nt : C1M_BLOCKS;
        hipStream_t st = (hipStream_t)stream;
        hipLaunchKernelGGL(conv_c1_wgrad_mfma_kernel, dim3(nblk, Cin / 32), dim3(C1_THREADS), 0, st, x, gy, workspace, B,
                           D, H, W, Cin, nDt, nHt, nWt, (int)nt);
        int rc = stx_check_launch("conv3d_c1_wgrad(mfma)");
        if (rc) return rc;
        hipLaunchKernelGGL(c1m_reduce_kernel, dim3(Cin * 27), dim3(C1_THREADS), 0, st, workspace, nblk, dw);
        return stx_check_launch("conv3d_c1_wgrad(reduce)");
    }
    C1Args a;
    a.x = x; a.w = nullptr; a.gy = gy; a.res = nullptr; a.out = workspace;
    a.B = B; a.D = D; a.H = H; a.W = W; a.Cin = Cin;
    a.nDt = stx_cdiv(D, C1_TD); a.nHt = stx_cdiv(H, C1_TH); a.nWt = stx_cdiv(W, C1_TW);
    a.ntiles = B * a.nDt * a.nHt * a.nWt;
    const int nblk = a.ntiles < C1_WGRAD_BLOCKS ? a.ntiles : C1_WGRAD_BLOCKS;
    const size_t lds = C1_TILE_BYTES + 256 * 4;
    hipStream_t st = (hipStream_t)stream;
    if (int rc = stx_lds_require((const void*)conv_c1_wgrad_kernel, lds, "conv3d_c1_wgrad")) return rc;
    hipLaunchKernelGGL(conv_c1_wgrad_kernel, dim3(nblk), dim3(C1_THREADS), lds, st, a);
    if (int rc = stx_check_launch("conv3d_c1_wgrad")) return rc;
    hipLaunchKernelGGL(c1_colsum_kernel, dim3(Cin * 27), dim3(C1_THREADS), 0, st, workspace, nblk, Cin * 27, dw);
    return stx_check_launch("conv3d_c1_colsum");
}

extern "C" int stx_conv3d_c1_dgrad(const float* gy, const float* w, float* gx, int B, int D, int H, int W, int Cin,
                                   void* stream) {
    stx_begin();
    STX_REQUIRE(gy && w && gx && B > 0 && D > 0 && H > 0 && W > 0, "conv3d_c1_dgrad: bad shape");
    STX_REQUIRE(Cin % 4 == 0 && Cin <= 64, "conv3d_c1_dgrad: Cin=%d must be a multiple of 4, <= 64", Cin);
    const int nHt = stx_cdiv(H, C1D_TH), nWt = stx_cdiv(W, C1D_TW);
    const long long nt = (long long)B * D * nHt * nWt;
    if (Cin == 32 && (long long)H * W * 128 < (1ll << 31) && nt < (1ll << 31)) {
        const long long g = nt < 256 * 8 ? nt : 256 * 8;
        hipLaunchKernelGGL(conv_c1_dgrad_mfma_kernel, dim3((unsigned)g), dim3(C1_THREADS), 0, (hipStream_t)stream, gy, w, gx, B, D,
                           H, W, nHt, nWt, (int)nt);
        return stx_check_launch("conv3d_c1_dgrad(mfma)");
    }
    hipLaunchKernelGGL(conv_c1_dgrad_kernel, dim3((unsigned)((size_t)B * D * nHt * nWt)), dim3(C1_THREADS), 0,
                       (hipStream_t)stream, gy, w, gx, B, D, H, W, Cin, nHt, nWt);
    return stx_check_launch("conv3d_c1_dgrad");
}
```

stereo_toolbox_amd/models/GwcNet/gwcnet.py:

```python
import torch
import torch.nn as nn

from ... import ops
from ...aggregation import conv_block, convbn_block, deferred_bn_counters, shared_input_convs
from ..features2d import ResTrunk, cat_features, channels_last_weights_, convbn, init_reference_style, run_head2d, run_pair
from .submodule import convbn_3d


class feature_extraction(ResTrunk):
    fused_everywhere = True

    def __init__(self, concat_feature=False, concat_feature_channel=12):
        super().__init__()
        self.concat_feature = concat_feature
        if concat_feature:
            self.lastconv = nn.Sequential(convbn(320, 128, 3, 1, 1, 1), nn.ReLU(inplace=True),
                                          nn.Conv2d(128, concat_feature_channel, 1, bias=False))

    def forward(self, x):
        gwc = cat_features(self.trunk(x))
        if not self.concat_feature:
            return {"gwc_feature": gwc}
        return {"gwc_feature": gwc, "concat_feature": run_head2d(self.lastconv, gwc)}


class hourglass(nn.Module):

    def __init__(self, c):
        super().__init__()
        self.conv1 = nn.Sequential(convbn_3d(c, c * 2, 3, 2, 1), nn.ReLU(inplace=True))
        self.conv2 = nn.Sequential(convbn_3d(c * 2, c * 2, 3, 1, 1), nn.ReLU(inplace=True))
        self.conv3 = nn.Sequential(convbn_3d(c * 2, c * 4, 3, 2, 1), nn.ReLU(inplace=True))
        self.conv4 = nn.Sequential(convbn_3d(c * 4, c * 4, 3, 1, 1), nn.ReLU(inplace=True))
        self.conv5 = nn.Sequential(nn.ConvTranspose3d(c * 4, c * 2, 3, padding=1, output_padding=1, stride=2, bias=False),
                                   nn.BatchNorm3d(c * 2))
        self.conv6 = nn.Sequential(nn.ConvTranspose3d(c * 2, c, 3, padding=1, output_padding=1, stride=2, bias=False),
                                   nn.BatchNorm3d(c))
        self.redir1 = convbn_3d(c, c, kernel_size=1, stride=1, pad=0)
        self.redir2 = convbn_3d(c * 2, c * 2, kernel_size=1, stride=1, pad=0)

    def forward(self, x, mid=None, also=None):
        rx = shared_input_convs(x, [self.conv1[0], self.redir1] + ([also] if also is not None else []))
        rx = rx or [None, None, None]
        c1 = convbn_block(x, self.conv1[0], relu=True, raw=rx[0])
        c2 = convbn_block(c1, self.conv2[0], relu=True)
        r2 = shared_input_convs(c2, [self.conv3[0], self.redir2]) or [None, None]
        c3 = convbn_block(c2, self.conv3[0], relu=True, raw=r2[0])
        c4 = convbn_block(c3, self.conv4[0], relu=True)
        if mid is not None:
            c4 = mid(c4)
        c5 = convbn_block(c4, self.conv5, relu=True, second=(c2, self.redir2), second_raw=r2[1])
        out = convbn_block(c5, self.conv6, relu=True, second=(x, self.redir1), second_raw=rx[1])
        return (out, rx[2]) if also is not None else out


def classifier(c):
    return nn.Sequential(convbn_3d(c, c, 3, 1, 1), nn.ReLU(inplace=True),
                         nn.Conv3d(c, 1, kernel_size=3, padding=1, stride=1, bias=False))


def run_classifier(seq, x, add=None, raw=None):
    h = convbn_block(x, seq[0], relu=True, raw=raw)
    cost = conv_block(h, seq[2], residual=None if add is None else add.unsqueeze(-1))
    return cost.squeeze(-1)


class GwcNet(nn.Module):
    def __init__(self, maxdisp, use_concat_volume=False):
        super().__init__()
        self.maxdisp = maxdisp
        self.use_concat_volume = use_concat_volume
        self.num_groups = 40
        if use_concat_volume:
            self.concat_channels = 12
            self.feature_extraction = feature_extraction(True, self.concat_channels)
        else:
            self.concat_channels = 0
            self.feature_extraction = feature_extraction(False)
        self.dres0 = nn.Sequential(convbn_3d(self.num_groups + self.concat_channels * 2, 32, 3, 1, 1),
                                   nn.ReLU(inplace=True), convbn_3d(32, 32, 3, 1, 1), nn.ReLU(inplace=True))
        self.dres1 = nn.Sequential(convbn_3d(32, 32, 3, 1, 1), nn.ReLU(inplace=True), convbn_3d(32, 32, 3, 1, 1))
        self.dres2 = hourglass(32)
        self.dres3 = hourglass(32)
        self.dres4 = hourglass(32)
        self.classif0 = classifier(32)
        self.classif1 = classifier(32)
        self.classif2 = classifier(32)
        self.classif3 = classifier(32)
        init_reference_style(self)
        channels_last_weights_(self.feature_extraction)

    def forward(self, left, right):
        with deferred_bn_counters():
            fl, fr = run_pair(self.feature_extraction, left, right, self.training)
            return self.aggregate(fl, fr, left.shape[2], left.shape[3])

    @ops.fp32_region
    def aggregate(self, fl, fr, H, W):
        vol = ops.cost_volume(fl["gwc_feature"], fr["gwc_feature"], fl.get("concat_feature"),
                              fr.get("concat_feature"), self.maxdisp // 4, self.num_groups, mask_left=True)
        cost0 = convbn_block(vol, self.dres0[0], relu=True)
        cost0 = convbn_block(cost0, self.dres0[2], relu=True)
        t = convbn_block(cost0, self.dres1[0], relu=True)
        cost0 = convbn_block(t, self.dres1[2], relu=False, residual=cost0)
        if self.training:
            out1, r0 = self.dres2(cost0, also=self.classif0[0])
            out2, r1 = self.dres3(out1, also=self.classif1[0])
            out3, r2 = self.dres4(out2, also=self.classif2[0])
            return [ops.regression_head(run_classifier(c, o, raw=r), self.maxdisp, H, W)
                    for c, o, r in ((self.classif0, cost0, r0), (self.classif1, out1, r1), (self.classif2, out2, r2),
                                    (self.classif3, out3, None))]
        out1 = self.dres2(cost0)
        out2 = self.dres3(out1)
        out3 = self.dres4(out2)
        return ops.regression_head(run_classifier(self.classif3, out3), self.maxdisp, H, W)


def GwcNet_G(d=192):
    return GwcNet(d, use_concat_volume=False)


def GwcNet_GC(d=192):
    return GwcNet(d, use_concat_volume=True)
```

stereo_toolbox_amd/ops.py:

```python
import ctypes

import torch

from ._capi import StxError, get_lib

_P = ctypes.c_void_p


class _DevPtr(ctypes.c_void_p):
    """A device pointer that remembers the device of the tensor it came from: _call() reads the launch device off its
    own arguments, so nothing survives between launches (an exception between building the arguments and the launch
    cannot leak state into the next one)."""


def _stream(dev=None):
    return _P(torch.cuda.current_stream(dev).cuda_stream)


def _p(t):
    if t is None:
        return None
    p = _DevPtr(t.data_ptr())
    p.dev = t.device
    return p


def on_device(t):
    return t.is_cuda


def _chk(t, name, dims=None):
    if t is None:
        return
    if not t.is_cuda:
        raise StxError(f"{name}: expected a ROCm device tensor, got {t.device} -- the cost-volume hot path has "
                       "no CPU fallback (the CPU oracle lives in oracle/ and is test-only)")
    if t.dtype != torch.float32:
        raise StxError(f"{name}: expected float32, got {t.dtype}")
    if not t.is_contiguous():
        raise StxError(f"{name}: expected a dense contiguous tensor, strides {t.stride()}")
    if dims is not None and t.dim() != dims:
        raise StxError(f"{name}: expected {dims} dims, got shape {tuple(t.shape)}")


def _call(name, *args):
    dev = None
    for a in args:
        if isinstance(a, _DevPtr):
            if dev is None:
                dev = a.dev
            elif a.dev != dev:
                raise StxError(f"{name}: operands live on different devices ({dev} and {a.dev})")
    if dev is not None and dev.type == "cuda" and dev.index != torch.cuda.current_device():
        with torch.cuda.device(dev):
            get_lib().call(name, *args, _stream(dev))
    else:
        get_lib().call(name, *args, _stream(dev))


_LOW = (torch.float16, torch.bfloat16)


def _to_fp32(v):
    if isinstance(v, torch.Tensor):
        return v.float() if v.dtype in _LOW else v
    if isinstance(v, dict):
        return {k: _to_fp32(x) for k, x in v.items()}
    if isinstance(v, (list, tuple)):
        return type(v)(_to_fp32(x) for x in v)
    return v


def autocast_active():
    return torch.is_autocast_enabled("cuda") or torch.is_autocast_enabled("cpu")


def fp32_region(fn):
    import functools

    @functools.wraps(fn)
    def wrapped(*args, **kwargs):
        if not autocast_active():
            return fn(*args, **kwargs)
        with torch.autocast("cuda", enabled=False), torch.autocast("cpu", enabled=False):
            return fn(*_to_fp32(args), **_to_fp32(kwargs))
    return wrapped


def to_ncdhw(x):
    return x.permute(0, 4, 1, 2, 3)


def to_ndhwc(x):
    return x.permute(0, 2, 3, 4, 1).contiguous()


class _Workspace:

    def __init__(self):
        self.bufs = {}

    def get(self, tag, nfloats, device):
        sid = torch.cuda.current_stream(device).cuda_stream if device.type == "cuda" else 0
        key = (device.index, sid, tag)
        b = self.bufs.get(key)
        if b is None or b.numel() < nfloats:
            b = torch.empty(int(nfloats), dtype=torch.float32, device=device)
            self.bufs[key] = b
        return b


_WS = _Workspace()


_CACHE_ENABLED = True


def set_weight_cache(enabled):
    global _CACHE_ENABLED
    _CACHE_ENABLED = bool(enabled)


def invalidate_caches(model):
    for m in model.modules():
        m.__dict__.pop("_stx_fold", None)
    for p in model.parameters():
        p.__dict__.pop("_stx_packed", None)


def pack_weight(w, mode, owner=None):
    _chk(w, "weight", 5)
    if owner is not None and _CACHE_ENABLED:
        cache = owner.__dict__.setdefault("_stx_packed", {})
        hit = cache.get(mode)
        if hit is not None and hit[0] == (owner._version, owner.data_ptr()):
            return hit[1]
    A, Bd = w.shape[0], w.shape[1]
    T = w.shape[2] * w.shape[3] * w.shape[4]
    K, N = (Bd, A) if mode == 0 else (A, Bd)
    n = get_lib().raw("stx_conv3d_packed_floats")(K, N, T)
    wp = torch.empty(n, dtype=torch.float32, device=w.device)
    _call("stx_conv3d_pack_weight", _p(w), _p(wp), A, Bd, T, mode)
    if owner is not None and _CACHE_ENABLED:
        cache[mode] = ((owner._version, owner.data_ptr()), wp)
    return wp


def _pad_channels(t, C):
    if t.shape[-1] == C:
        return t
    out = t.new_zeros(*t.shape[:-1], C)
    out[..., : t.shape[-1]] = t
    return out


def pad_input_channels(x, w):
    Cin = x.shape[-1]
    Cp = (Cin + 7) // 8 * 8
    if Cp == Cin:
        return x, w
    wp = w.new_zeros(w.shape[0], Cp, *w.shape[2:])
    wp[:, :Cin] = w
    return _pad_channels(x, Cp), wp


def pad_weight_channels(w, Cp):
    if w.shape[1] == Cp:
        return w
    wp = w.new_zeros(w.shape[0], Cp, *w.shape[2:])
    wp[:, : w.shape[1]] = w
    return wp


def conv_out_dims(D, H, W, ks, stride):
    pad = ks // 2
    return tuple((d + 2 * pad - ks) // stride + 1 for d in (D, H, W))


def conv3d_forward(x, wp, Cout, ks, stride, scale=None, bias=None, residual=None, relu=False, want_stats=False):
    _chk(x, "x", 5)
    B, D, H, W, Cin = x.shape
    Do, Ho, Wo = conv_out_dims(D, H, W, ks, stride)
    out = torch.empty(B, Do, Ho, Wo, Cout, dtype=torch.float32, device=x.device)
    stats = None
    if want_stats:
        rows = get_lib().raw("stx_conv3d_fwd_stat_rows")(B, D, H, W, Cin, Cout, ks, stride)
        stats = torch.empty(rows, 2, Cout, dtype=torch.float32, device=x.device)
    _call("stx_conv3d_fwd", _p(x), _p(wp), _p(out), _p(scale), _p(bias), _p(residual), _p(stats), B, D, H, W, Cin,
          Cout, ks, stride, int(relu))
    return out, stats


def deconv3d_forward(x, wp, Cout, out_dims=None, scale=None, bias=None, residual=None, relu=False, want_stats=False):
    _chk(x, "x", 5)
    B, D, H, W, Cin = x.shape
    Do, Ho, Wo = out_dims if out_dims is not None else (2 * D, 2 * H, 2 * W)
    if Cout > 64:
        if Cout % 64 != 0:
            raise StxError(f"deconv3d_forward: Cout={Cout} > 64 must be a multiple of 64")
        nt = Cout // 32
        wv = wp.view(-1, Cin // 8, nt, 256)
        outs, sts = [], []
        for h in range(Cout // 64):
            sl = slice(64 * h, 64 * h + 64)
            o, st_ = deconv3d_forward(x, wv[:, :, 2 * h:2 * h + 2].contiguous(), 64, (Do, Ho, Wo),
                                      None if scale is None else scale[sl].contiguous(),
                                      None if bias is None else bias[sl].contiguous(),
                                      None if residual is None else residual[..., sl].contiguous(), relu, want_stats)
            outs.append(o)
            sts.append(st_)
        return torch.cat(outs, -1), (torch.cat(sts, -1) if want_stats else None)
    out = torch.empty(B, Do, Ho, Wo, Cout, dtype=torch.float32, device=x.device)
    stats = None
    if want_stats:
        nb = get_lib().raw("stx_deconv3d_fwd_blocks")(D, H, W)
        stats = torch.empty(B * nb, 2, Cout, dtype=torch.float32, device=x.device)
    _call("stx_deconv3d_fwd", _p(x), _p(wp), _p(out), _p(scale), _p(bias), _p(residual), _p(stats), B, D, H, W, Cin,
          Cout, Do, Ho, Wo, int(relu))
    return out, stats


def conv3d_wgrad(fine, coarse, ks, stride):
    B, Df, Hf, Wf, CF = fine.shape
    _, Dc, Hc, Wc, CC = coarse.shape
    n = get_lib().raw("stx_conv3d_wgrad_workspace_floats")(B, Dc, Hc, Wc, CF, CC, ks, stride)
    ws = _WS.get("wgrad", n, fine.device)
    dw = torch.empty(CC, CF, ks ** 3, dtype=torch.float32, device=fine.device)
    _call("stx_conv3d_wgrad", _p(fine), _p(coarse), _p(dw), _p(ws), B, Df, Hf, Wf, CF, Dc, Hc, Wc, CC, ks, stride)
    return dw


def conv3d_wgrad_bn(x, gy, pend):
    B, D, H, W, CF = x.shape
    CC = gy.shape[-1]
    n = get_lib().raw("stx_conv3d_wgrad_workspace_floats")(B, D, H, W, CF, CC, 3, 1)
    ws = _WS.get("wgrad", n, x.device)
    dw = torch.empty(CC, CF, 27, dtype=torch.float32, device=x.device)
    dz = torch.empty_like(gy)
    _call("stx_conv3d_wgrad_bn", _p(x), _p(gy), _p(pend.z), _p(pend.scale), _p(pend.shift), _p(pend.mean), _p(pend.invstd),
          _p(pend.gamma), _p(pend.sums), float(pend.inv_n), int(pend.act), _p(dz), _p(dw), _p(ws), B, D, H, W, CF, CC)
    return dw, dz


class _PendingBn:
    __slots__ = ("g", "z", "scale", "shift", "mean", "invstd", "gamma", "sums", "inv_n", "act")

    def materialize(self):
        C = self.z.shape[-1]
        nvox = self.z.numel() // C
        dz = torch.empty_like(self.z)
        _call("stx_bn_bwd_apply2", _p(self.g), None, _p(self.z), _p(self.mean), _p(self.invstd), _p(self.gamma), None, None,
              None, None, _p(self.scale), _p(self.shift), None, None, _p(self.sums), _p(dz), None, None, nvox, C, int(self.act), 1)
        return dz


_BN_DEFER = {"outstanding": 0, "armed": False}


def _bn_defer_check():
    n, _BN_DEFER["outstanding"], _BN_DEFER["armed"] = _BN_DEFER["outstanding"], 0, False
    if n:
        raise StxError(f"{n} deferred BatchNorm-backward record(s) were not consumed by their convolution's backward node: "
                       "the gradients of this backward pass are wrong (set STX_BN_BWD_IN_WGRAD=0 and report)")


def _defer_pending_bn(g, pend):
    g._stx_pending_bn = pend
    _BN_DEFER["outstanding"] += 1
    if not _BN_DEFER["armed"]:
        _BN_DEFER["armed"] = True
        torch.autograd.Variable._execution_engine.queue_callback(_bn_defer_check)


def bn_defer_reset_if_stale():
    if not _BN_DEFER["armed"]:
        return
    task_id = getattr(torch._C, "_current_graph_task_id", None)
    if task_id is None or task_id() == -1:
        _BN_DEFER["outstanding"], _BN_DEFER["armed"] = 0, False


def _take_pending_bn(g):
    pend = getattr(g, "_stx_pending_bn", None) if g is not None else None
    if pend is not None:
        del g._stx_pending_bn
        _BN_DEFER["outstanding"] -= 1
        if pend.g is not g:
            raise StxError("deferred BatchNorm backward: record attached to a different gradient tensor")
    return pend


def _is_c1(w, ks, stride, transposed):
    return (not transposed) and ks == 3 and stride == 1 and w.shape[0] == 1 and w.shape[1] % 16 == 0 and w.shape[1] <= 64


def conv3d_c1_forward(x, w, residual=None):
    _chk(x, "x", 5)
    _chk(w, "weight", 5)
    B, D, H, W, Cin = x.shape
    out = torch.empty(B, D, H, W, 1, dtype=torch.float32, device=x.device)
    _call("stx_conv3d_c1_fwd", _p(x), _p(w), _p(residual), _p(out), B, D, H, W, Cin)
    return out


def conv3d_c1_wgrad(x, gy):
    B, D, H, W, Cin = x.shape
    ws = _WS.get("c1wgrad", get_lib().raw("stx_conv3d_c1_wgrad_workspace_floats")(Cin), x.device)
    dw = torch.empty(1, Cin, 3, 3, 3, dtype=torch.float32, device=x.device)
    _call("stx_conv3d_c1_wgrad", _p(x), _p(gy), _p(dw), _p(ws), B, D, H, W, Cin)
    return dw


def conv3d_c1_dgrad(gy, w, Cin):
    B, D, H, W, _ = gy.shape
    gx = torch.empty(B, D, H, W, Cin, dtype=torch.float32, device=gy.device)
    _call("stx_conv3d_c1_dgrad", _p(gy), _p(w), _p(gx), B, D, H, W, Cin)
    return gx


class ConvRawFn(torch.autograd.Function):

    @staticmethod
    def forward(ctx, x, w, ks, stride, transposed, want_stats):
        _chk(x, "x", 5)
        ctx.cin_true = None
        ctx.x_prepadded = False
        if not transposed and x.shape[-1] != w.shape[1]:
            if x.shape[-1] != (w.shape[1] + 7) // 8 * 8:
                raise StxError(f"conv: input has {x.shape[-1]} channels, weight expects {w.shape[1]}")
            ctx.cin_true, ctx.x_prepadded = w.shape[1], True
            w = pad_weight_channels(w, x.shape[-1])
        elif not transposed and x.shape[-1] % 8 != 0:
            ctx.cin_true = x.shape[-1]
            x, w = pad_input_channels(x, w)
        if _is_c1(w, ks, stride, transposed) and not want_stats:
            z, stats = conv3d_c1_forward(x, w.contiguous()), None
        elif transposed:
            Cout = w.shape[1]
            z, stats = deconv3d_forward(x, pack_weight(w, 2), Cout, want_stats=want_stats)
        else:
            Cout = w.shape[0]
            z, stats = conv3d_forward(x, pack_weight(w, 0), Cout, ks, stride, want_stats=want_stats)
        ctx.save_for_backward(x, w)
        ctx.cfg = (ks, stride, transposed)
        if stats is None:
            stats = x.new_empty(0)
        ctx.mark_non_differentiable(stats)
        return z, stats

    @staticmethod
    def backward(ctx, gz, _gstats):
        x, w = ctx.saved_tensors
        ks, stride, transposed = ctx.cfg
        pend = _take_pending_bn(gz)
        gx = gw = None
        B, D, H, W, Cin = x.shape
        if pend is not None:
            if (ctx.needs_input_grad[1] and not transposed and ks == 3 and stride == 1 and ctx.cin_true is None
                    and get_lib().raw("stx_conv3d_wgrad_bn_supported")(B, D, H, W, Cin, w.shape[0])):
                gw_pre, gz = conv3d_wgrad_bn(x, gz, pend)
                gw_pre = gw_pre.reshape(w.shape)
            else:
                gw_pre, gz = None, pend.materialize()
        else:
            gw_pre = None
        gz = gz.contiguous()
        if transposed:
            Ci, Co = w.shape[0], w.shape[1]
            if ctx.needs_input_grad[0]:
                gx, _ = conv3d_forward(gz, pack_weight(w, 0), Ci, 3, 2)
            if ctx.needs_input_grad[1]:
                gz_w = gz if Co % 32 == 0 else _pad_channels(gz, (Co + 31) // 32 * 32)
                x_w = x if Ci % 32 == 0 else _pad_channels(x, (Ci + 31) // 32 * 32)
                gw = conv3d_wgrad(gz_w, x_w, 3, 2)[:Ci, :Co].reshape(w.shape)
        else:
            Co, Ci = w.shape[0], w.shape[1]
            c1 = _is_c1(w, ks, stride, transposed)
            gz_k, w_k = gz, w
            if Co % 8 != 0 and not c1:
                Cp = (Co + 7) // 8 * 8
                gz_k = _pad_channels(gz, Cp)
                w_k = w.new_zeros(Cp, *w.shape[1:])
                w_k[:Co] = w
            if ctx.needs_input_grad[0]:
                if c1:
                    gx = conv3d_c1_dgrad(gz, w.contiguous(), Ci)
                elif stride == 1 and Ci > 128:
                    parts = []
                    for lo in range(0, Ci, 128):
                        hi = min(Ci, lo + 128)
                        g, _ = conv3d_forward(gz_k, pack_weight(w_k[:, lo:hi].contiguous(), 1), hi - lo, ks, 1)
                        parts.append(g)
                    gx = torch.cat(parts, -1)
                elif stride == 1:
                    gx, _ = conv3d_forward(gz_k, pack_weight(w_k, 1), Ci, ks, 1)
                else:
                    if Co % 32:
                        Cp = (Co + 31) // 32 * 32
                        gz_k = _pad_channels(gz, Cp)
                        w_k = w.new_zeros(Cp, *w.shape[1:])
                        w_k[:Co] = w
                    gx, _ = deconv3d_forward(gz_k, pack_weight(w_k, 2), Ci, out_dims=(D, H, W))
            if gw_pre is not None:
                gw = gw_pre
            elif ctx.needs_input_grad[1]:
                if c1:
                    gw = conv3d_c1_wgrad(x, gz)
                else:
                    gz_w = gz if Co % 32 == 0 else _pad_channels(gz, (Co + 31) // 32 * 32)
                    x_w = x if Ci % 32 == 0 else _pad_channels(x, (Ci + 31) // 32 * 32)
                    gw = conv3d_wgrad(x_w, gz_w, ks, stride)[:Co, :Ci].reshape(w.shape)
        if ctx.cin_true is not None:
            if gx is not None and not ctx.x_prepadded:
                gx = gx[..., :ctx.cin_true].contiguous()
            if gw is not None:
                gw = gw[:, :ctx.cin_true].contiguous()
        return gx, gw, None, None, None, None


class SharedInputConvsFn(torch.autograd.Function):

    @staticmethod
    def forward(ctx, x, cfgs, *ws):
        _chk(x, "x", 5)
        outs = []
        for (ks, stride, want), w in zip(cfgs, ws):
            if x.shape[-1] != w.shape[1] or w.shape[1] % 8 or w.shape[0] % 8 or _is_c1(w, ks, stride, False):
                raise StxError(f"SharedInputConvsFn: weight {tuple(w.shape)} on an input of {x.shape[-1]} channels")
            z, stats = conv3d_forward(x, pack_weight(w, 0), w.shape[0], ks, stride, want_stats=want)
            if stats is None:
                stats = x.new_empty(0)
            ctx.mark_non_differentiable(stats)
            outs += [z, stats]
        ctx.save_for_backward(x, *ws)
        ctx.cfgs = cfgs
        return tuple(outs)

    @staticmethod
    def backward(ctx, *grads):
        x, ws = ctx.saved_tensors[0], ctx.saved_tensors[1:]
        B, D, H, W, Ci = x.shape
        gws = [None] * len(ws)
        gzs = []
        for k, g in enumerate(grads[0::2]):
            pend = _take_pending_bn(g)
            if pend is not None:
                ks, stride, _ = ctx.cfgs[k]
                if (ctx.needs_input_grad[2 + k] and ks == 3 and stride == 1
                        and get_lib().raw("stx_conv3d_wgrad_bn_supported")(B, D, H, W, Ci, ws[k].shape[0])):
                    gw, g = conv3d_wgrad_bn(x, g, pend)
                    gws[k] = gw.reshape(ws[k].shape)
                else:
                    g = pend.materialize()
            gzs.append(None if g is None else g.contiguous())
        gx = None
        if ctx.needs_input_grad[0]:
            rank = lambda k: (0 if ctx.cfgs[k][0] == 3 and ctx.cfgs[k][1] == 1 else (1 if ctx.cfgs[k][1] == 2 else 2))
            for k in sorted((k for k in range(len(ws)) if gzs[k] is not None), key=rank):
                (ks, stride, _), w, gz = ctx.cfgs[k], ws[k], gzs[k]
                if stride == 1:
                    gx, _ = conv3d_forward(gz, pack_weight(w, 1), Ci, ks, 1, residual=gx)
                else:
                    Co = w.shape[0]
                    gz_k, w_k = gz, w
                    if Co % 32:
                        Cp = (Co + 31) // 32 * 32
                        gz_k = _pad_channels(gz, Cp)
                        w_k = w.new_zeros(Cp, *w.shape[1:])
                        w_k[:Co] = w
                    gx, _ = deconv3d_forward(gz_k, pack_weight(w_k, 2), Ci, out_dims=(D, H, W), residual=gx)
        for k, (w, gz) in enumerate(zip(ws, gzs)):
            if gz is None or not ctx.needs_input_grad[2 + k] or gws[k] is not None:
                continue
            ks, stride, _ = ctx.cfgs[k]
            Co = w.shape[0]
            gz_w = gz if Co % 32 == 0 else _pad_channels(gz, (Co + 31) // 32 * 32)
            x_w = x if Ci % 32 == 0 else _pad_channels(x, (Ci + 31) // 32 * 32)
            gws[k] = conv3d_wgrad(x_w, gz_w, ks, stride)[:Co, :Ci].reshape(w.shape)
        return (gx, None, *gws)


_D4_SEL = ((3, 1, 4), (4, 2, 0))


def embed_deconv4_weight(w):
    Ci, Co = w.shape[0], w.shape[1]
    wz = torch.cat((w, w.new_zeros(Ci, Co, 1, 4, 4)), 2)
    wz = torch.cat((wz, wz.new_zeros(Ci, Co, 5, 1, 4)), 3)
    wz = torch.cat((wz, wz.new_zeros(Ci, Co, 5, 5, 1)), 4)
    parts = []
    for pd in (0, 1):
        for ph in (0, 1):
            for pw in (0, 1):
                sel = wz[:, :, list(_D4_SEL[pd])][:, :, :, list(_D4_SEL[ph])][:, :, :, :, list(_D4_SEL[pw])]
                parts.append(sel.transpose(0, 1))
    return torch.cat(parts, 0).contiguous()


class DepthToSpaceFn(torch.autograd.Function):

    @staticmethod
    def forward(ctx, y):
        y = y.contiguous()
        _chk(y, "y", 5)
        B, D, H, W, C8 = y.shape
        C = C8 // 8
        out = torch.empty(B, 2 * D, 2 * H, 2 * W, C, dtype=torch.float32, device=y.device)
        _call("stx_depth_to_space", _p(y), _p(out), B, D, H, W, C, 0)
        return out

    @staticmethod
    def backward(ctx, g):
        g = g.contiguous()
        B, D2, H2, W2, C = g.shape
        gy = torch.empty(B, D2 // 2, H2 // 2, W2 // 2, 8 * C, dtype=torch.float32, device=g.device)
        _call("stx_depth_to_space", _p(g), _p(gy), B, D2 // 2, H2 // 2, W2 // 2, C, 1)
        return gy


def _d4_chunks(Co):
    per = max(1, min(8, 128 // Co))
    return [(c0, min(8, c0 + per)) for c0 in range(0, 8, per)]


def deconv4_raw(x, w, want_stats):
    Co = w.shape[1]
    if Co % 4:
        raise StxError(f"ConvTranspose3d(k4): {Co} output channels (need a multiple of 4)")
    w3 = embed_deconv4_weight(w)
    ys = [ConvRawFn.apply(x, w3[c0 * Co:c1 * Co], 3, 1, False, False)[0] for c0, c1 in _d4_chunks(Co)]
    z = DepthToSpaceFn.apply(ys[0] if len(ys) == 1 else torch.cat(ys, -1))
    return z, (bn_stats(z.detach()) if want_stats else z.new_empty(0))


@fp32_region
def deconv4_forward(x, w, scale=None, bias=None, relu=0, owner=None):
    _chk(x, "x", 5)
    Co = w.shape[1]
    if Co % 4:
        raise StxError(f"ConvTranspose3d(k4): {Co} output channels (need a multiple of 4)")
    cache = owner.__dict__.setdefault("_stx_packed", {}) if (owner is not None and _CACHE_ENABLED) else None
    key = (owner._version, owner.data_ptr()) if owner is not None else None
    hit = cache.get("d4") if cache is not None else None
    if hit is not None and hit[0] == key:
        packed = hit[1]
    else:
        w3 = embed_deconv4_weight(w)
        packed = [pack_weight(w3[c0 * Co:c1 * Co].contiguous(), 0) for c0, c1 in _d4_chunks(Co)]
        if cache is not None:
            cache["d4"] = (key, packed)
    ys = []
    for (c0, c1), wp in zip(_d4_chunks(Co), packed):
        n = c1 - c0
        ys.append(conv3d_forward(x, wp, n * Co, 3, 1, None if scale is None else scale.repeat(n),
                                 None if bias is None else bias.repeat(n), None, relu)[0])
    B, D, H, W, _ = x.shape
    y = ys[0] if len(ys) == 1 else torch.cat(ys, -1)
    out = torch.empty(B, 2 * D, 2 * H, 2 * W, Co, dtype=torch.float32, device=x.device)
    _call("stx_depth_to_space", _p(y), _p(out), B, D, H, W, Co, 0)
    return out


class GateFn(torch.autograd.Function):

    @staticmethod
    def forward(ctx, cv, att):
        out = gate(cv.detach(), att.detach())
        ctx.save_for_backward(cv, att)
        return out

    @staticmethod
    def backward(ctx, g):
        cv, att = ctx.saved_tensors
        g = g.contiguous()
        B, D, H, W, C = cv.shape
        gcv = torch.empty_like(cv) if ctx.needs_input_grad[0] else None
        gatt = torch.empty_like(att) if ctx.needs_input_grad[1] else None
        if gcv is not None or gatt is not None:
            _call("stx_gate_bwd", _p(g), _p(cv), _p(att), _p(gcv), _p(gatt), B, D, H * W, C)
        return gcv, gatt


@fp32_region
def gate(cv, att):
    if torch.is_grad_enabled() and (cv.requires_grad or att.requires_grad):
        return GateFn.apply(cv.contiguous(), att.contiguous())
    cv, att = cv.contiguous(), att.contiguous()
    _chk(cv, "cv", 5)
    _chk(att, "att", 4)
    B, D, H, W, C = cv.shape
    if att.shape != (B, H, W, C) or C % 4:
        raise StxError(f"gate: volume {tuple(cv.shape)} vs gate {tuple(att.shape)} (need [B,H,W,C], C % 4 == 0)")
    out = torch.empty_like(cv)
    _call("stx_gate_fwd", _p(cv), _p(att), _p(out), B, D, H * W, C)
    return out


class ChannelMajorFn(torch.autograd.Function):

    @staticmethod
    def forward(ctx, x):
        B, C, H, W = x.shape
        out = torch.empty((B, C, H, W), dtype=x.dtype, device=x.device)
        _call("stx_transpose", _p(x.permute(0, 2, 3, 1)), _p(out), B, H * W, C)
        return out

    @staticmethod
    def backward(ctx, g):
        g = g.contiguous()
        B, C, H, W = g.shape
        gx = torch.empty((B, H, W, C), dtype=g.dtype, device=g.device)
        _call("stx_transpose", _p(g), _p(gx), B, C, H * W)
        return gx.permute(0, 3, 1, 2)


@fp32_region
def channel_major(x):
    if x.is_contiguous():
        return x
    if (x.dim() == 4 and x.dtype == torch.float32 and on_device(x) and x.is_contiguous(memory_format=torch.channels_last)
# ... 1528 lines not shown
```

Baseline: 0.1786 pairs/s.

## Fuse classifier BN+ReLU into single-channel 3D conv fwd, wgrad and dgrad

After: 0.1786 pairs/s, median of 3. About the same (+0.0%).

```diff
diff --git a/include/stx_hip.h b/include/stx_hip.h
--- a/include/stx_hip.h
+++ b/include/stx_hip.h
@@ -65,6 +65,16 @@
 int stx_conv3d_c1_wgrad(const float* x, const float* gy, float* dw, float* workspace, int B, int D, int H, int W,
                         int Cin, void* stream);
 int stx_conv3d_c1_dgrad(const float* gy, const float* w, float* gx, int B, int D, int H, int W, int Cin, void* stream);
+
+int stx_conv3d_c1_bn_supported(int B, int D, int H, int W, int Cin);
+int stx_conv3d_c1_fwd_bn(const float* z, const float* scale, const float* shift, const float* w, const float* residual,
+                         float* out, int B, int D, int H, int W, int Cin, void* stream);
+int stx_conv3d_c1_wgrad_bn(const float* z, const float* scale, const float* shift, const float* gy, float* dw,
+                           float* workspace, int B, int D, int H, int W, int Cin, void* stream);
+int stx_conv3d_c1_dgrad_bn_rows(void);
+int stx_conv3d_c1_dgrad_bn(const float* gy, const float* w, const float* z, const float* scale, const float* shift,
+                           const float* mean, const float* invstd, float* gx, float* partials, float* sums, int B, int D,
+                           int H, int W, int Cin, void* stream);
 
 int stx_mish_fwd(const float* x, float* y, long long n, void* stream);
 int stx_mish_bwd(const float* gy, const float* x, float* gx, long long n, void* stream);
@@ -108,6 +118,7 @@
                      const float* gamma1, const float* z2, const float* mean2, const float* invstd2,
                      const float* gamma2, const float* sums, float* dz1, float* dz2, float* gout, long long nvox, int C,
                      int relu, void* stream);
+int stx_bn_colsum(const float* partials, int nrows, int M, float* sums, void* stream);
 int stx_bn_bwd_reduce2(const float* gy, const float* y, const float* z1, const float* mean1, const float* invstd1,
                        const float* z2, const float* mean2, const float* invstd2, const float* scale1,
                        const float* shift1, const float* scale2, const float* shift2, float* partials, float* sums,
diff --git a/stereo_toolbox_amd/_capi.py b/stereo_toolbox_amd/_capi.py
--- a/stereo_toolbox_amd/_capi.py
+++ b/stereo_toolbox_amd/_capi.py
@@ -47,6 +47,11 @@
     "stx_conv3d_c1_wgrad_workspace_floats": [_I],
     "stx_conv3d_c1_wgrad": [_P, _P, _P, _P, _I, _I, _I, _I, _I, _P],
     "stx_conv3d_c1_dgrad": [_P, _P, _P, _I, _I, _I, _I, _I, _P],
+    "stx_conv3d_c1_bn_supported": [_I, _I, _I, _I, _I],
+    "stx_conv3d_c1_fwd_bn": [_P, _P, _P, _P, _P, _P, _I, _I, _I, _I, _I, _P],
+    "stx_conv3d_c1_wgrad_bn": [_P, _P, _P, _P, _P, _P, _I, _I, _I, _I, _I, _P],
+    "stx_conv3d_c1_dgrad_bn_rows": [],
+    "stx_conv3d_c1_dgrad_bn": [_P] * 10 + [_I, _I, _I, _I, _I, _P],
     "stx_mish_fwd": [_P, _P, _L, _P],
     "stx_mish_bwd": [_P, _P, _P, _L, _P],
     "stx_depth_to_space": [_P, _P, _I, _I, _I, _I, _I, _I, _P],
@@ -114,6 +119,7 @@
     "stx_bn_bwd_reduce": [_P, _P, _P, _P, _P, _P, _P, _P, _P, _P, _L, _I, _I, _P],
     "stx_bn_bwd_apply": [_P, _P, _P, _P, _P, _P, _P, _P, _P, _P, _P, _P, _P, _P, _L, _I, _I, _P],
     "stx_bn_bwd_reduce2": [_P] * 14 + [_L, _I, _I, _I, _P],
+    "stx_bn_colsum": [_P, _I, _I, _P, _P],
     "stx_bn_bwd_apply2": [_P] * 18 + [_L, _I, _I, _I, _P],
 }
 _RET_CHARP = ("stx_last_error", "stx_build_info")
diff --git a/stereo_toolbox_amd/aggregation.py b/stereo_toolbox_amd/aggregation.py
--- a/stereo_toolbox_amd/aggregation.py
+++ b/stereo_toolbox_amd/aggregation.py
@@ -211,6 +211,30 @@
 
 
 @ops.fp32_region
+def classifier_head(x, seq, tail, add=None, raw=None):
+    fuse_fwd, fuse_bwd = ops.c1_bn_fuse()
+    conv, bn = seq[0], seq[1]
+    if not (fuse_fwd or fuse_bwd) or not torch.is_grad_enabled() or not bn.training or isinstance(bn, nn.SyncBatchNorm):
+        return None
+    if bn.weight is None or bn.bias is None or tail.bias is not None or _is_transposed(conv) or _is_transposed(tail):
+        return None
+    if tuple(tail.weight.shape) != (1, 32, 3, 3, 3) or conv.weight.shape[0] != 32 or tail.stride[0] != 1 or tail.padding[0] != 1:
+        return None
+    if not all(p.requires_grad for p in (conv.weight, bn.weight, bn.bias, tail.weight)):
+        return None
+    z, part = raw if raw is not None else _raw_conv(x, conv, True)
+    if not z.requires_grad or not ops.conv3d_c1_bn_supported(z):
+        h = conv_block(x, conv, bn, relu=True, raw=(z, part))
+        return conv_block(h, tail, residual=add)
+    st = _bn_state(bn, part, z.numel() // z.shape[-1])
+    defer = (_conv_cfg(conv) == (3, 1) and conv.weight.shape[1] % 32 == 0
+             and os.environ.get("STX_BN_BWD_IN_WGRAD", "1") != "0")
+    if defer:
+        ops.bn_defer_reset_if_stale()
+    return ops.C1HeadFn.apply(z, bn.weight, bn.bias, tail.weight, add, st, defer, fuse_fwd, fuse_bwd)
+
+
+@ops.fp32_region
 def convbn_block(x, seq, relu=False, second=None, residual=None, mish=False, raw=None, second_raw=None):
     sec = None
     if second is not None:
diff --git a/stereo_toolbox_amd/csrc/bn.hip b/stereo_toolbox_amd/csrc/bn.hip
--- a/stereo_toolbox_amd/csrc/bn.hip
+++ b/stereo_toolbox_amd/csrc/bn.hip
@@ -433,6 +433,13 @@
     return stx_check_launch("bn_colsum");
 }
 
+extern "C" int stx_bn_colsum(const float* partials, int nrows, int M, float* sums, void* stream) {
+    stx_begin();
+    STX_REQUIRE(partials && sums && nrows > 0 && M > 0, "bn_colsum: bad args");
+    hipLaunchKernelGGL(bn_colsum_kernel, dim3(M), dim3(BN_THREADS), 0, (hipStream_t)stream, partials, nrows, M, sums, 1);
+    return stx_check_launch("bn_colsum");
+}
+
 extern "C" int stx_bn_bwd_apply2(const float* gy, const float* y, const float* z1, const float* mean1,
                                  const float* invstd1, const float* gamma1, const float* z2, const float* mean2,
                                  const float* invstd2, const float* gamma2, const float* scale1, const float* shift1,
diff --git a/stereo_toolbox_amd/csrc/conv_c1.hip b/stereo_toolbox_amd/csrc/conv_c1.hip
--- a/stereo_toolbox_amd/csrc/conv_c1.hip
+++ b/stereo_toolbox_amd/csrc/conv_c1.hip
@@ -146,6 +146,7 @@
 
 constexpr int C1D_TH = 4, C1D_TW = 32;
 constexpr int C1D_EH = C1D_TH + 2, C1D_EW = C1D_TW + 2;
+constexpr int C1D_WGS = 256 * 8;
 
 __global__ __launch_bounds__(C1_THREADS) void conv_c1_dgrad_kernel(const float* __restrict__ gy,
                                                                    const float* __restrict__ w, float* __restrict__ gx,
@@ -209,12 +210,22 @@
 }
 
 
+template <bool BN>
 __global__ __launch_bounds__(C1_THREADS) void conv_c1_dgrad_mfma_kernel(const float* __restrict__ gy,
                                                                         const float* __restrict__ w, float* __restrict__ gx,
+                                                                        const float* __restrict__ z,
+                                                                        const float* __restrict__ scale,
+                                                                        const float* __restrict__ shift,
+                                                                        const float* __restrict__ mean,
+                                                                        const float* __restrict__ invstd,
+                                                                        float* __restrict__ partials,
                                                                         int B, int D, int H, int W, int nHt, int nWt, int ntiles) {
     __shared__ float gys[3 * C1D_EH * C1D_EW];
     const int tid = threadIdx.x, lane = tid & 63, wave = tid >> 6;
     const int i = lane & 31, half = lane >> 5;
+    float bsc = 0.f, bsh = 0.f, bmu = 0.f, bis = 0.f;
+    double sg = 0.0, sgx = 0.0;
+    if constexpr (BN) { bsc = scale[i]; bsh = shift[i]; bmu = mean[i]; bis = invstd[i]; }
     float wreg[14];
     int aoff[14];
 #pragma unroll
@@ -233,6 +244,18 @@
         const int d = r_ % D;
         const int b = r_ / D;
         const int h0 = ht * C1D_TH, w0 = wt * C1D_TW;
+        const int oh = h0 + wave;
+        const unsigned vbase = (unsigned)((((oh < H ? oh : 0) * W + w0 + 4 * half) * 32 + i) * 4);
+        float zv[16];
+        if constexpr (BN) {
+            const stx_bufrsrc zrs = stx_make_rsrc(z + ((size_t)b * D + d) * H * W * 32, plane_bytes);
+#pragma unroll
+            for (int r = 0; r < 16; ++r) {
+                const int m = (r & 3) + 8 * (r >> 2);
+                const bool ok = oh < H && w0 + 4 * half + m < W;
+                zv[r] = stx_buf_ld1(zrs, ok ? vbase : STX_BUF_OOB, (unsigned)(m * 128));
+            }
+        }
         __syncthreads();
         for (int idx = tid; idx < 3 * C1D_EH * C1D_EW; idx += C1_THREADS) {
             const int wx = idx % C1D_EW, hy = (idx / C1D_EW) % C1D_EH, dz = idx / (C1D_EW * C1D_EH);
@@ -249,15 +272,37 @@
         for (int j = 0; j < 14; ++j) av[j] = gys[aoff[j]];
 #pragma unroll
         for (int j = 0; j < 14; ++j) acc = __builtin_amdgcn_mfma_f32_32x32x2f32(av[j], wreg[j], acc, 0, 0, 0);
-        const int oh = h0 + wave;
         const stx_bufrsrc ors = stx_make_rsrc(gx + ((size_t)b * D + d) * H * W * 32, plane_bytes);
-        const unsigned vbase = (unsigned)((((oh < H ? oh : 0) * W + w0 + 4 * half) * 32 + i) * 4);
 #pragma unroll
         for (int r = 0; r < 16; ++r) {
             const int m = (r & 3) + 8 * (r >> 2);
             const bool ok = oh < H && w0 + 4 * half + m < W;
             stx_buf_st1(ors, ok ? vbase : STX_BUF_OOB, (unsigned)(m * 128), acc[r]);
         }
+        if constexpr (BN) {
+#pragma unroll
+            for (int r = 0; r < 16; ++r) {
+                const int m = (r & 3) + 8 * (r >> 2);
+                const bool ok = oh < H && w0 + 4 * half + m < W;
+                const float g = ok ? stx_act_bwd(acc[r], fmaf(zv[r], bsc, bsh), 1) : 0.f;
+                const float xh = (zv[r] - bmu) * bis;
+                sg += (double)g;
+                sgx = fma((double)g, (double)xh, sgx);
+            }
+        }
+    }
+    if constexpr (BN) {
+        __shared__ double red[2][8][32];
+        red[0][2 * wave + half][i] = sg;
+        red[1][2 * wave + half][i] = sgx;
+        __syncthreads();
+        if (tid < 64) {
+            const int k = tid >> 5, c = tid & 31;
+            double t = 0.0;
+#pragma unroll
+            for (int j = 0; j < 8; ++j) t += red[k][j][c];
+            partials[((size_t)blockIdx.x * 2 + k) * 32 + c] = (float)t;
+        }
     }
 }
 
@@ -266,8 +311,11 @@
 constexpr int C1M_ED = C1M_TD + 2, C1M_EH = C1M_TH + 2, C1M_EW = C1M_TW + 2;
 constexpr int C1M_BLOCKS = 1024;
 
+template <bool BN>
 __global__ __launch_bounds__(C1_THREADS) void conv_c1_wgrad_mfma_kernel(const float* __restrict__ x,
                                                                         const float* __restrict__ gy,
+                                                                        const float* __restrict__ scale,
+                                                                        const float* __restrict__ shift,
                                                                         float* __restrict__ slab, int B, int D, int H,
                                                                         int W, int Cin, int nDt, int nHt, int nWt,
                                                                         int ntiles) {
@@ -276,6 +324,8 @@
     const int tid = threadIdx.x, lane = tid & 63, wave = tid >> 6;
     const int i = lane & 31, half = lane >> 5;
     const int cb = blockIdx.y;
+    float bsc = 0.f, bsh = 0.f;
+    if constexpr (BN) { bsc = scale[cb * 32 + i]; bsh = shift[cb * 32 + i]; }
     const int kd = i / 9, kh = (i / 3) % 3, kw = i % 3;
     const int toff = (i < 27) ? ((2 - kd) * C1M_EH + (2 - kh)) * C1M_EW + (2 - kw) + half : half;
     f32x16 acc;
@@ -307,6 +357,11 @@
 #pragma unroll
             for (int p = 0; p < 16; ++p)
                 av[p] = (rowok && w0 + 2 * p + half < W) ? xr[(size_t)(2 * p) * Cin] : 0.f;
+            if constexpr (BN) {
+#pragma unroll
+                for (int p = 0; p < 16; ++p)
+                    av[p] = (rowok && w0 + 2 * p + half < W) ? stx_act(fmaf(av[p], bsc, bsh), 1) : 0.f;
+            }
             const float* gp = gys + (ld * C1M_EH + lh) * C1M_EW + toff;
 #pragma unroll
             for (int p = 0; p < 16; ++p) {
@@ -347,9 +402,12 @@
 constexpr int C1F_MT = (C1F_NV + 31) / 32;
 constexpr int C1F_WGS = 512;
 
+template <bool BN>
 __global__ __launch_bounds__(C1_THREADS) void conv_c1_fwd_mfma_kernel(const float* __restrict__ x,
                                                                       const float* __restrict__ w,
                                                                       const float* __restrict__ res,
+                                                                      const float* __restrict__ scale,
+                                                                      const float* __restrict__ shift,
                                                                       float* __restrict__ out, int B, int D, int H, int W,
                                                                       int nHt, int nWt, int ncols) {
     STX_DYN_SMEM(smem);
@@ -359,6 +417,11 @@
     float wreg[16];
 #pragma unroll
     for (int s_ = 0; s_ < 16; ++s_) wreg[s_] = (i < 27) ? w[(size_t)(16 * half + s_) * 27 + i] : 0.f;
+    float bsc[16], bsh[16];
+    if constexpr (BN) {
+#pragma unroll
+        for (int s_ = 0; s_ < 16; ++s_) { bsc[s_] = scale[16 * half + s_]; bsh[s_] = shift[16 * half + s_]; }
+    }
     const int lh = tid / C1F_TW, lw = tid % C1F_TW;
 
     constexpr int MTW = (C1F_MT + 3) / 4;
@@ -416,10 +479,18 @@
                         for (int r = 0; r < 16; ++r) acc[r] = 0.f;
 #pragma unroll
                         for (int q = 0; q < 4; ++q) {
-                            acc = __builtin_amdgcn_mfma_f32_32x32x2f32(cur[t][q].x, wreg[4 * q + 0], acc, 0, 0, 0);
-                            acc = __builtin_amdgcn_mfma_f32_32x32x2f32(cur[t][q].y, wreg[4 * q + 1], acc, 0, 0, 0);
-                            acc = __builtin_amdgcn_mfma_f32_32x32x2f32(cur[t][q].z, wreg[4 * q + 2], acc, 0, 0, 0);
-                            acc = __builtin_amdgcn_mfma_f32_32x32x2f32(cur[t][q].w, wreg[4 * q + 3], acc, 0, 0, 0);
+                            float4 a4 = cur[t][q];
+                            if constexpr (BN) {
+                                const bool vok = voff[t] != STX_BUF_OOB;
+                                a4.x = vok ? stx_act(fmaf(a4.x, bsc[4 * q + 0], bsh[4 * q + 0]), 1) : 0.f;
+                                a4.y = vok ? stx_act(fmaf(a4.y, bsc[4 * q + 1], bsh[4 * q + 1]), 1) : 0.f;
+                                a4.z = vok ? stx_act(fmaf(a4.z, bsc[4 * q + 2], bsh[4 * q + 2]), 1) : 0.f;
+                                a4.w = vok ? stx_act(fmaf(a4.w, bsc[4 * q + 3], bsh[4 * q + 3]), 1) : 0.f;
+                            }
+                            acc = __builtin_amdgcn_mfma_f32_32x32x2f32(a4.x, wreg[4 * q + 0], acc, 0, 0, 0);
+                            acc = __builtin_amdgcn_mfma_f32_32x32x2f32(a4.y, wreg[4 * q + 1], acc, 0, 0, 0);
+                            acc = __builtin_amdgcn_mfma_f32_32x32x2f32(a4.z, wreg[4 * q + 2], acc, 0, 0, 0);
+                            acc = __builtin_amdgcn_mfma_f32_32x32x2f32(a4.w, wreg[4 * q + 3], acc, 0, 0, 0);
                         }
                         if (i < 27) {
 #pragma unroll
@@ -458,23 +529,32 @@
 
 }
 
+static bool c1_mfma_shape(int B, int D, int H, int W, int Cin) {
+    return B > 0 && D > 0 && H > 0 && W > 0 && Cin == 32 && (long long)H * W * 128 < (1ll << 31);
+}
+
+template <bool BN>
+static int c1_fwd_mfma_launch(const float* x, const float* w, const float* residual, const float* scale, const float* shift,
+                              float* out, int B, int D, int H, int W, void* stream) {
+    const int nHt = stx_cdiv(H, C1F_TH), nWt = stx_cdiv(W, C1F_TW);
+    const long long ncols = (long long)B * nHt * nWt, units = ncols * D;
+    STX_REQUIRE(units < (1ll << 31), "conv3d_c1_fwd: volume too large");
+    long long g = C1F_WGS;
+    if (g > units / 4) g = units / 4 > 0 ? units / 4 : 1;
+    const size_t lds = (size_t)2 * C1F_NV * 27 * 4;
+    if (int rc = stx_lds_require((const void*)conv_c1_fwd_mfma_kernel<BN>, lds, "conv3d_c1_fwd(mfma)")) return rc;
+    hipLaunchKernelGGL((conv_c1_fwd_mfma_kernel<BN>), dim3((unsigned)g), dim3(C1_THREADS), lds, (hipStream_t)stream, x, w,
+                       residual, scale, shift, out, B, D, H, W, nHt, nWt, (int)ncols);
+    return stx_check_launch("conv3d_c1_fwd(mfma)");
+}
+
 extern "C" int stx_conv3d_c1_fwd(const float* x, const float* w, const float* residual, float* out, int B, int D,
                                  int H, int W, int Cin, void* stream) {
     stx_begin();
     STX_REQUIRE(x && w && out && B > 0 && D > 0 && H > 0 && W > 0, "conv3d_c1_fwd: bad shape");
     STX_REQUIRE(Cin % C1_CK == 0, "conv3d_c1_fwd: Cin=%d must be a multiple of %d", Cin, C1_CK);
-    if (Cin == 32 && (long long)H * W * 128 < (1ll << 31)) {
-        const int nHt = stx_cdiv(H, C1F_TH), nWt = stx_cdiv(W, C1F_TW);
-        const long long ncols = (long long)B * nHt * nWt, units = ncols * D;
-        STX_REQUIRE(units < (1ll << 31), "conv3d_c1_fwd: volume too large");
-        long long g = C1F_WGS;
-        if (g > units / 4) g = units / 4 > 0 ? units / 4 : 1;
-        const size_t lds = (size_t)2 * C1F_NV * 27 * 4;
-        if (int rc = stx_lds_require((const void*)conv_c1_fwd_mfma_kernel, lds, "conv3d_c1_fwd(mfma)")) return rc;
-        hipLaunchKernelGGL(conv_c1_fwd_mfma_kernel, dim3((unsigned)g), dim3(C1_THREADS), lds, (hipStream_t)stream, x, w,
-                           residual, out, B, D, H, W, nHt, nWt, (int)ncols);
-        return stx_check_launch("conv3d_c1_fwd(mfma)");
-    }
+    if (c1_mfma_shape(B, D, H, W, Cin))
+        return c1_fwd_mfma_launch<false>(x, w, residual, nullptr, nullptr, out, B, D, H, W, stream);
     C1Args a;
     a.x = x; a.w = w; a.gy = nullptr; a.res = residual; a.out = out;
     a.B = B; a.D = D; a.H = H; a.W = W; a.Cin = Cin;
@@ -491,24 +571,29 @@
     return valu > mfma ? valu : mfma;
 }
 
+template <bool BN>
+static int c1_wgrad_mfma_launch(const float* x, const float* gy, const float* scale, const float* shift, float* dw,
+                                float* workspace, int B, int D, int H, int W, int Cin, void* stream) {
+    const int nDt = stx_cdiv(D, C1M_TD), nHt = stx_cdiv(H, C1M_TH), nWt = stx_cdiv(W, C1M_TW);
+    const long long nt = (long long)B * nDt * nHt * nWt;
+    STX_REQUIRE(nt < (1ll << 31), "conv3d_c1_wgrad: volume too large");
+    const int nblk = nt < C1M_BLOCKS ? (int)nt : C1M_BLOCKS;
+    hipStream_t st = (hipStream_t)stream;
+    hipLaunchKernelGGL((conv_c1_wgrad_mfma_kernel<BN>), dim3(nblk, Cin / 32), dim3(C1_THREADS), 0, st, x, gy, scale, shift,
+                       workspace, B, D, H, W, Cin, nDt, nHt, nWt, (int)nt);
+    int rc = stx_check_launch("conv3d_c1_wgrad(mfma)");
+    if (rc) return rc;
+    hipLaunchKernelGGL(c1m_reduce_kernel, dim3(Cin * 27), dim3(C1_THREADS), 0, st, workspace, nblk, dw);
+    return stx_check_launch("conv3d_c1_wgrad(reduce)");
+}
+
 extern "C" int stx_conv3d_c1_wgrad(const float* x, const float* gy, float* dw, float* workspace, int B, int D, int H,
                                    int W, int Cin, void* stream) {
     stx_begin();
     STX_REQUIRE(x && gy && dw && workspace && B > 0, "conv3d_c1_wgrad: null operand");
     STX_REQUIRE(Cin % C1_CK == 0 && Cin <= 4 * C1_CK, "conv3d_c1_wgrad: Cin=%d must be 16..64 in steps of 16", Cin);
-    if (Cin % 32 == 0) {
-        const int nDt = stx_cdiv(D, C1M_TD), nHt = stx_cdiv(H, C1M_TH), nWt = stx_cdiv(W, C1M_TW);
-        const long long nt = (long long)B * nDt * nHt * nWt;
-        STX_REQUIRE(nt < (1ll << 31), "conv3d_c1_wgrad: volume too large");
-        const int nblk = nt < C1M_BLOCKS ? (int)nt : C1M_BLOCKS;
-        hipStream_t st = (hipStream_t)stream;
-        hipLaunchKernelGGL(conv_c1_wgrad_mfma_kernel, dim3(nblk, Cin / 32), dim3(C1_THREADS), 0, st, x, gy, workspace, B,
-                           D, H, W, Cin, nDt, nHt, nWt, (int)nt);
-        int rc = stx_check_launch("conv3d_c1_wgrad(mfma)");
-        if (rc) return rc;
-        hipLaunchKernelGGL(c1m_reduce_kernel, dim3(Cin * 27), dim3(C1_THREADS), 0, st, workspace, nblk, dw);
-        return stx_check_launch("conv3d_c1_wgrad(reduce)");
-    }
+    if (Cin % 32 == 0)
+        return c1_wgrad_mfma_launch<false>(x, gy, nullptr, nullptr, dw, workspace, B, D, H, W, Cin, stream);
     C1Args a;
     a.x = x; a.w = nullptr; a.gy = gy; a.res = nullptr; a.out = workspace;
     a.B = B; a.D = D; a.H = H; a.W = W; a.Cin = Cin;
@@ -532,12 +617,52 @@
     const int nHt = stx_cdiv(H, C1D_TH), nWt = stx_cdiv(W, C1D_TW);
     const long long nt = (long long)B * D * nHt * nWt;
     if (Cin == 32 && (long long)H * W * 128 < (1ll << 31) && nt < (1ll << 31)) {
-        const long long g = nt < 256 * 8 ? nt : 256 * 8;
-        hipLaunchKernelGGL(conv_c1_dgrad_mfma_kernel, dim3((unsigned)g), dim3(C1_THREADS), 0, (hipStream_t)stream, gy, w, gx, B, D,
-                           H, W, nHt, nWt, (int)nt);
+        const long long g = nt < C1D_WGS ? nt : C1D_WGS;
+        hipLaunchKernelGGL((conv_c1_dgrad_mfma_kernel<false>), dim3((unsigned)g), dim3(C1_THREADS), 0, (hipStream_t)stream, gy,
+                           w, gx, nullptr, nullptr, nullptr, nullptr, nullptr, nullptr, B, D, H, W, nHt, nWt, (int)nt);
         return stx_check_launch("conv3d_c1_dgrad(mfma)");
     }
     hipLaunchKernelGGL(conv_c1_dgrad_kernel, dim3((unsigned)((size_t)B * D * nHt * nWt)), dim3(C1_THREADS), 0,
                        (hipStream_t)stream, gy, w, gx, B, D, H, W, Cin, nHt, nWt);
     return stx_check_launch("conv3d_c1_dgrad");
 }
+
+extern "C" int stx_conv3d_c1_bn_supported(int B, int D, int H, int W, int Cin) {
+    const long long nt = (long long)B * D * stx_cdiv(H, C1D_TH) * stx_cdiv(W, C1D_TW);
+    return c1_mfma_shape(B, D, H, W, Cin) && nt < (1ll << 31);
+}
+
+extern "C" int stx_conv3d_c1_fwd_bn(const float* z, const float* scale, const float* shift, const float* w,
+                                    const float* residual, float* out, int B, int D, int H, int W, int Cin, void* stream) {
+    stx_begin();
+    STX_REQUIRE(z && scale && shift && w && out, "conv3d_c1_fwd_bn: null operand");
+    STX_REQUIRE(stx_conv3d_c1_bn_supported(B, D, H, W, Cin), "conv3d_c1_fwd_bn: shape [%d,%d,%d,%d,%d] not served", B, D, H, W, Cin);
+    return c1_fwd_mfma_launch<true>(z, w, residual, scale, shift, out, B, D, H, W, stream);
+}
+
+extern "C" int stx_conv3d_c1_wgrad_bn(const float* z, const float* scale, const float* shift, const float* gy, float* dw,
+                                      float* workspace, int B, int D, int H, int W, int Cin, void* stream) {
+    stx_begin();
+    STX_REQUIRE(z && scale && shift && gy && dw && workspace, "conv3d_c1_wgrad_bn: null operand");
+    STX_REQUIRE(stx_conv3d_c1_bn_supported(B, D, H, W, Cin), "conv3d_c1_wgrad_bn: shape [%d,%d,%d,%d,%d] not served", B, D, H, W, Cin);
+    return c1_wgrad_mfma_launch<true>(z, gy, scale, shift, dw, workspace, B, D, H, W, Cin, stream);
+}
+
+extern "C" int stx_conv3d_c1_dgrad_bn_rows(void) { return C1D_WGS; }
+
+extern "C" int stx_bn_colsum(const float* partials, int nrows, int M, float* sums, void* stream);
+
+extern "C" int stx_conv3d_c1_dgrad_bn(const float* gy, const float* w, const float* z, const float* scale,
+                                      const float* shift, const float* mean, const float* invstd, float* gx,
+                                      float* partials, float* sums, int B, int D, int H, int W, int Cin, void* stream) {
+    stx_begin();
+    STX_REQUIRE(gy && w && z && scale && shift && mean && invstd && gx && partials && sums, "conv3d_c1_dgrad_bn: null operand");
+    STX_REQUIRE(stx_conv3d_c1_bn_supported(B, D, H, W, Cin), "conv3d_c1_dgrad_bn: shape [%d,%d,%d,%d,%d] not served", B, D, H, W, Cin);
+    const int nHt = stx_cdiv(H, C1D_TH), nWt = stx_cdiv(W, C1D_TW);
+    const long long nt = (long long)B * D * nHt * nWt;
+    const int g = (int)(nt < C1D_WGS ? nt : C1D_WGS);
+    hipLaunchKernelGGL((conv_c1_dgrad_mfma_kernel<true>), dim3((unsigned)g), dim3(C1_THREADS), 0, (hipStream_t)stream, gy, w, gx,
+                       z, scale, shift, mean, invstd, partials, B, D, H, W, nHt, nWt, (int)nt);
+    if (int rc = stx_check_launch("conv3d_c1_dgrad_bn")) return rc;
+    return stx_bn_colsum(partials, g, 64, sums, stream);
+}
diff --git a/stereo_toolbox_amd/models/GwcNet/gwcnet.py b/stereo_toolbox_amd/models/GwcNet/gwcnet.py
--- a/stereo_toolbox_amd/models/GwcNet/gwcnet.py
+++ b/stereo_toolbox_amd/models/GwcNet/gwcnet.py
@@ -2,7 +2,7 @@
 import torch.nn as nn
 
 from ... import ops
-from ...aggregation import conv_block, convbn_block, deferred_bn_counters, shared_input_convs
+from ...aggregation import classifier_head, conv_block, convbn_block, deferred_bn_counters, shared_input_convs
 from ..features2d import ResTrunk, cat_features, channels_last_weights_, convbn, init_reference_style, run_head2d, run_pair
 from .submodule import convbn_3d
 
@@ -60,8 +60,11 @@
 
 
 def run_classifier(seq, x, add=None, raw=None):
-    h = convbn_block(x, seq[0], relu=True, raw=raw)
-    cost = conv_block(h, seq[2], residual=None if add is None else add.unsqueeze(-1))
+    res = None if add is None else add.unsqueeze(-1)
+    cost = classifier_head(x, seq[0], seq[2], add=res, raw=raw)
+    if cost is None:
+        h = convbn_block(x, seq[0], relu=True, raw=raw)
+        cost = conv_block(h, seq[2], residual=res)
     return cost.squeeze(-1)
 
 
diff --git a/stereo_toolbox_amd/ops.py b/stereo_toolbox_amd/ops.py
--- a/stereo_toolbox_amd/ops.py
+++ b/stereo_toolbox_amd/ops.py
@@ -1,4 +1,5 @@
 import ctypes
+import os
 
 import torch
 
@@ -316,6 +317,112 @@
     gx = torch.empty(B, D, H, W, Cin, dtype=torch.float32, device=gy.device)
     _call("stx_conv3d_c1_dgrad", _p(gy), _p(w), _p(gx), B, D, H, W, Cin)
     return gx
+
+
+def _parse_c1_bn_fuse(v):
+    v = v.strip().lower()
+    return {"fwd": v in ("1", "fwd"), "bwd": v in ("1", "bwd")}
+
+
+_C1_BN_FUSE = _parse_c1_bn_fuse(os.environ.get("STX_C1_BN_FUSE", "1"))
+
+
+def set_c1_bn_fuse(fwd=None, bwd=None):
+    old = (_C1_BN_FUSE["fwd"], _C1_BN_FUSE["bwd"])
+    if fwd is not None:
+        _C1_BN_FUSE["fwd"] = bool(fwd)
+    if bwd is not None:
+        _C1_BN_FUSE["bwd"] = bool(bwd)
+    return old
+
+
+def c1_bn_fuse():
+    return _C1_BN_FUSE["fwd"], _C1_BN_FUSE["bwd"]
+
+
+def conv3d_c1_bn_supported(z):
+    B, D, H, W, C = z.shape
+    return bool(get_lib().raw("stx_conv3d_c1_bn_supported")(B, D, H, W, C))
+
+
+def conv3d_c1_forward_bn(z, scale, shift, w, residual=None):
+    _chk(z, "z", 5)
+    _chk(w, "weight", 5)
+    B, D, H, W, Cin = z.shape
+    out = torch.empty(B, D, H, W, 1, dtype=torch.float32, device=z.device)
+    _call("stx_conv3d_c1_fwd_bn", _p(z), _p(scale), _p(shift), _p(w), _p(residual), _p(out), B, D, H, W, Cin)
+    return out
+
+
+def conv3d_c1_wgrad_bn(z, scale, shift, gy):
+    B, D, H, W, Cin = z.shape
+    ws = _WS.get("c1wgrad", get_lib().raw("stx_conv3d_c1_wgrad_workspace_floats")(Cin), z.device)
+    dw = torch.empty(1, Cin, 3, 3, 3, dtype=torch.float32, device=z.device)
+    _call("stx_conv3d_c1_wgrad_bn", _p(z), _p(scale), _p(shift), _p(gy), _p(dw), _p(ws), B, D, H, W, Cin)
+    return dw
+
+
+def conv3d_c1_dgrad_bn(gy, w, z, scale, shift, mean, invstd, sums):
+    B, D, H, W, Cin = z.shape
+    part = _WS.get("c1bnred", get_lib().raw("stx_conv3d_c1_dgrad_bn_rows")() * 2 * Cin, z.device)
+    gx = torch.empty_like(z)
+    _call("stx_conv3d_c1_dgrad_bn", _p(gy), _p(w), _p(z), _p(scale), _p(shift), _p(mean), _p(invstd), _p(gx), _p(part),
+          _p(sums), B, D, H, W, Cin)
+    return gx
+
+
+class C1HeadFn(torch.autograd.Function):
+
+    @staticmethod
+    def forward(ctx, z, gamma, beta, w, residual, bn, defer, fuse_fwd, fuse_bwd):
+        _chk(z, "z", 5)
+        w = w.contiguous()
+        sc, sh, m, i = bn_finalize(bn["partials"], bn["count"], gamma, beta, bn["running_mean"], bn["running_var"],
+                                   bn["momentum"], bn["eps"])
+        if residual is not None:
+            residual = residual.contiguous()
+        if fuse_fwd:
+            y = None
+            out = conv3d_c1_forward_bn(z, sc, sh, w, residual)
+        else:
+            y = bn_apply(z, sc, sh, None, None, None, 1)
+            out = conv3d_c1_forward(y, w, residual)
+        ctx.save_for_backward(z, gamma, m, i, sc, sh, w, y)
+        ctx.defer, ctx.fuse_bwd, ctx.has_res = bool(defer), bool(fuse_bwd), residual is not None
+        return out
+
+    @staticmethod
+    def backward(ctx, gout):
+        z, gamma, m, i, sc, sh, w, y = ctx.saved_tensors
+        gout = gout.contiguous()
+        C = z.shape[-1]
+        nvox = z.numel() // C
+        gw = None
+        if ctx.needs_input_grad[3]:
+            gw = conv3d_c1_wgrad(y, gout) if y is not None else conv3d_c1_wgrad_bn(z, sc, sh, gout)
+        sums = torch.empty(1, 3, C, dtype=torch.float32, device=z.device)
+        if ctx.fuse_bwd:
+            gy = conv3d_c1_dgrad_bn(gout, w, z, sc, sh, m, i, sums)
+        else:
+            gy = conv3d_c1_dgrad(gout, w, C)
+            part = _WS.get("bnred", get_lib().raw("stx_bn_reduce_blocks")() * 3 * C, z.device)
+            _call("stx_bn_bwd_reduce2", _p(gy), None, _p(z), _p(m), _p(i), None, None, None, _p(sc), _p(sh), None, None,
+                  _p(part), _p(sums), nvox, C, 1, 1)
+        gres = gout if ctx.has_res else None
+        tot = sums[0]
+        if not ctx.needs_input_grad[0]:
+            return (None, tot[1], tot[0], gw, gres, None, None, None, None)
+        if ctx.defer:
+            alias = gy.view_as(gy)
+            pend = _PendingBn()
+            pend.g, pend.z, pend.scale, pend.shift, pend.mean, pend.invstd = alias, z, sc, sh, m, i
+            pend.gamma, pend.sums, pend.inv_n, pend.act = gamma, sums, 1.0 / nvox, 1
+            _defer_pending_bn(alias, pend)
+            return (alias, tot[1], tot[0], gw, gres, None, None, None, None)
+        dz = torch.empty_like(z)
+        _call("stx_bn_bwd_apply2", _p(gy), None, _p(z), _p(m), _p(i), _p(gamma), None, None, None, None, _p(sc), _p(sh), None,
+              None, _p(sums), _p(dz), None, None, nvox, C, 1, 1)
+        return (dz, tot[1], tot[0], gw, gres, None, None, None, None)
 
 
 class ConvRawFn(torch.autograd.Function):
```
